# wangjiarui153/AIGV-Assessor

Measured on AMD Instinct MI355X. Metric: scored clips/sec (8-frame 448x448, InternVL2-8B stage-2 score eval), higher is better.
Workload: dtype bf16

## Files before the change

### aigv-assessor_amd/csrc/slowfast.hip

```cpp
#include <hip/hip_runtime.h>

#include <algorithm>
#include <cmath>
#include <cstdarg>
#include <cstdio>
#include <cstring>
#include <map>
#include <string>
#include <vector>

#include "../../include/aigv_amd.h"
#include "common.h"
#include "kernels.h"

namespace {

struct ConvArgs {
  const bf16_t* in;
  const bf16_t* w;
  const float* bias;
  const bf16_t* res;
  bf16_t* out;
  int ld_in, Cin, Ti, Hi, Wi;
  int kt, kh, kw, st, sh, sw, pt, ph, pw;
  int To, Ho, Wo, Cout, CoutPad, Kp;
  int ld_res, ld_out, c_off, relu;
  long rows;
  float* part;
  int k_slices;
};

template <int BN>
__global__ __launch_bounds__(256) void conv3d_mfma_kernel(ConvArgs p) {
  constexpr int BM = 128, BK = 64, NT = BN / 16, WJ = (BN + 31) / 32;
  __shared__ __attribute__((aligned(16))) bf16_t sA[BM * BK];
  __shared__ __attribute__((aligned(16))) bf16_t sW[BN * BK];
  const int tid = threadIdx.x, lane = tid & 63, wave = tid >> 6;
  const long m0 = (long)blockIdx.x * BM;
  const int n0 = blockIdx.y * BN;
  const int kspan = p.Kp / p.k_slices, kb = blockIdx.z * kspan;
  const int kc = tid & 7;
  const int r0 = tid >> 3;
  long base[4];
  int t0[4], y0[4], x0[4];
  bool rv[4];
#pragma unroll
  for (int j = 0; j < 4; ++j) {
    const long m = m0 + r0 + 32 * j;
    rv[j] = m < p.rows;
    const long mm = rv[j] ? m : 0;
    const int x = (int)(mm % p.Wo);
    const long r1 = mm / p.Wo;
    const int y = (int)(r1 % p.Ho);
    const long r2 = r1 / p.Ho;
    const int t = (int)(r2 % p.To);
    const long b = r2 / p.To;
    t0[j] = t * p.st - p.pt;
    y0[j] = y * p.sh - p.ph;
    x0[j] = x * p.sw - p.pw;
    base[j] = b * p.Ti * p.Hi * p.Wi;
  }
  int c = kb + kc * 8, dx = 0, dy = 0, dt = 0;
  auto normalise = [&]() {
    while (c >= p.Cin) {
      c -= p.Cin;
      if (++dx == p.kw) {
        dx = 0;
        if (++dy == p.kh) { dy = 0; ++dt; }
      }
    }
  };
  normalise();
  auto gather = [&](int j) -> u16x8 {
    u16x8 z = {0, 0, 0, 0, 0, 0, 0, 0};
    if (!rv[j] || dt >= p.kt) return z;
    const int tt = t0[j] + dt, yy = y0[j] + dy, xx = x0[j] + dx;
    if ((unsigned)tt >= (unsigned)p.Ti || (unsigned)yy >= (unsigned)p.Hi || (unsigned)xx >= (unsigned)p.Wi) return z;
    return *(const u16x8*)(p.in + (base[j] + ((long)tt * p.Hi + yy) * p.Wi + xx) * p.ld_in + c);
  };
  bool wv[WJ];
  const bf16_t* wsrc[WJ];
#pragma unroll
  for (int j = 0; j < WJ; ++j) {
    const int wrow = r0 + 32 * j;
    wv[j] = wrow < BN && (n0 + wrow) < p.CoutPad;
    wsrc[j] = p.w + (size_t)(n0 + (wv[j] ? wrow : 0)) * p.Kp + kb + kc * 8;
  }
  f32x4 acc[2][NT];
#pragma unroll
  for (int i = 0; i < 2; ++i)
#pragma unroll
    for (int n = 0; n < NT; ++n) acc[i][n] = f32x4{0.f, 0.f, 0.f, 0.f};

  const u16x8 zero = {0, 0, 0, 0, 0, 0, 0, 0};
  u16x8 ra[4], rw[WJ];
#pragma unroll
  for (int j = 0; j < 4; ++j) ra[j] = gather(j);
#pragma unroll
  for (int j = 0; j < WJ; ++j) rw[j] = wv[j] ? *(const u16x8*)wsrc[j] : zero;
  const int slot = (kc ^ (r0 & 7)) * 8;
  for (int k0 = 0; k0 < kspan; k0 += BK) {
    __syncthreads();
#pragma unroll
    for (int j = 0; j < 4; ++j) *(u16x8*)&sA[(r0 + 32 * j) * BK + slot] = ra[j];
#pragma unroll
    for (int j = 0; j < WJ; ++j)
      if (r0 + 32 * j < BN) *(u16x8*)&sW[(r0 + 32 * j) * BK + slot] = rw[j];
    __syncthreads();
    if (k0 + BK < kspan) {
      c += BK;
      normalise();
#pragma unroll
      for (int j = 0; j < 4; ++j) ra[j] = gather(j);
#pragma unroll
      for (int j = 0; j < WJ; ++j) rw[j] = wv[j] ? *(const u16x8*)(wsrc[j] + k0 + BK) : zero;
    }
#pragma unroll
    for (int h = 0; h < 2; ++h) {
      const int rs = ((h * 4 + (lane >> 4)) ^ (lane & 7)) * 8;
      bf16x8 a[2], w[NT];
#pragma unroll
      for (int i = 0; i < 2; ++i) a[i] = *(const bf16x8*)&sA[(wave * 32 + i * 16 + (lane & 15)) * BK + rs];
#pragma unroll
      for (int n = 0; n < NT; ++n) w[n] = *(const bf16x8*)&sW[(n * 16 + (lane & 15)) * BK + rs];
#pragma unroll
      for (int i = 0; i < 2; ++i)
#pragma unroll
        for (int n = 0; n < NT; ++n) acc[i][n] = __builtin_amdgcn_mfma_f32_16x16x32_bf16(w[n], a[i], acc[i][n], 0, 0, 0);
    }
  }
#pragma unroll
  for (int i = 0; i < 2; ++i) {
    const long m = m0 + wave * 32 + i * 16 + (lane & 15);
    if (m >= p.rows) continue;
#pragma unroll
    for (int n = 0; n < NT; ++n) {
      const int ch = n0 + n * 16 + (lane >> 4) * 4;
      if (ch >= p.Cout) continue;
      if (p.k_slices > 1) {
        *(f32x4*)(p.part + ((size_t)blockIdx.z * p.rows + m) * p.Cout + ch) = acc[i][n];
        continue;
      }
      float v[4];
#pragma unroll
      for (int e = 0; e < 4; ++e) v[e] = acc[i][n][e] + p.bias[ch + e];
      if (p.res) {
        const u16x4 r = *(const u16x4*)(p.res + m * p.ld_res + ch);
#pragma unroll
        for (int e = 0; e < 4; ++e) v[e] += bf2f(r[e]);
      }
      u16x4 o;
#pragma unroll
      for (int e = 0; e < 4; ++e) o[e] = f2bf(p.relu ? fmaxf(v[e], 0.f) : v[e]);
      *(u16x4*)(p.out + m * p.ld_out + p.c_off + ch) = o;
    }
  }
}

__global__ __launch_bounds__(256) void conv_finalize_kernel(ConvArgs p) {
  const long i = (long)blockIdx.x * 256 + threadIdx.x;
  const int cq = p.Cout >> 2;
  if (i >= p.rows * cq) return;
  const long m = i / cq;
  const int ch = (int)(i - m * cq) * 4;
  f32x4 v = *(const f32x4*)(p.part + (size_t)m * p.Cout + ch);
  for (int z = 1; z < p.k_slices; ++z) v += *(const f32x4*)(p.part + ((size_t)z * p.rows + m) * p.Cout + ch);
#pragma unroll
  for (int e = 0; e < 4; ++e) v[e] += p.bias[ch + e];
  if (p.res) {
    const u16x4 r = *(const u16x4*)(p.res + m * p.ld_res + ch);
#pragma unroll
    for (int e = 0; e < 4; ++e) v[e] += bf2f(r[e]);
  }
  u16x4 o;
#pragma unroll
  for (int e = 0; e < 4; ++e) o[e] = f2bf(p.relu ? fmaxf(v[e], 0.f) : v[e]);
  *(u16x4*)(p.out + m * p.ld_out + p.c_off + ch) = o;
}

struct FrameIdx { int v[64]; };
__global__ __launch_bounds__(256) void sf_repack_kernel(const bf16_t* __restrict__ frames, int T, int Ts, long hw, bf16_t* __restrict__ fast,
                                                        bf16_t* __restrict__ slow, FrameIdx idx, long total) {
  const long i = (long)blockIdx.x * 256 + threadIdx.x;
  if (i >= total) return;
  const long px = i % hw;
  const long f = i / hw;
  const int tt = (int)(f % (T + Ts));
  const long b = f / (T + Ts);
  const int src_t = tt < T ? tt : idx.v[tt - T];
  const bf16_t* s = frames + ((b * T + src_t) * 3) * hw + px;
  u16x4 o = {s[0], s[hw], s[2 * hw], 0};
  bf16_t* d = tt < T ? fast + ((b * T + tt) * hw + px) * 4 : slow + ((b * Ts + (tt - T)) * hw + px) * 4;
  *(u16x4*)d = o;
}

__global__ __launch_bounds__(256) void sf_maxpool_kernel(const bf16_t* __restrict__ in, int C, int Hi, int Wi, int Ho, int Wo,
                                                         bf16_t* __restrict__ out, int ld_out, long total) {
  const long i = (long)blockIdx.x * 256 + threadIdx.x;
  if (i >= total) return;
  const int cv = C >> 3;
  const int c8 = (int)(i % cv);
  const long px = i / cv;
  const int x = (int)(px % Wo);
  const long r = px / Wo;
  const int y = (int)(r % Ho);
  const long f = r / Ho;
  float m[8];
#pragma unroll
  for (int e = 0; e < 8; ++e) m[e] = -INFINITY;
  for (int dy = 0; dy < 3; ++dy) {
    const int yy = 2 * y - 1 + dy;
    if ((unsigned)yy >= (unsigned)Hi) continue;
    for (int dx = 0; dx < 3; ++dx) {
      const int xx = 2 * x - 1 + dx;
      if ((unsigned)xx >= (unsigned)Wi) continue;
      const u16x8 v = *(const u16x8*)(in + ((f * Hi + yy) * Wi + xx) * C + c8 * 8);
#pragma unroll
      for (int e = 0; e < 8; ++e) m[e] = fmaxf(m[e], bf2f(v[e]));
    }
  }
  u16x8 o;
#pragma unroll
  for (int e = 0; e < 8; ++e) o[e] = f2bf(m[e]);
  *(u16x8*)(out + px * ld_out + c8 * 8) = o;
}

struct PoolW { float t[32], y[32], x[32]; };
__global__ __launch_bounds__(256) void sf_pool_kernel(const bf16_t* __restrict__ in, int T, int H, int W, int C, PoolW w,
                                                      bf16_t* __restrict__ out, int ld_out, int c_off) {
  __shared__ float red[64][4][8];
  const int chunk = threadIdx.x & 3, slice = threadIdx.x >> 2;
  const int c8 = blockIdx.x * 4 + chunk;
  const int b = blockIdx.y;
  float acc[8] = {0.f, 0.f, 0.f, 0.f, 0.f, 0.f, 0.f, 0.f};
  if (c8 * 8 < C) {
    const bf16_t* s = in + (long)b * T * H * W * C + c8 * 8;
    const int n = T * H * W;
    for (int i = slice; i < n; i += 64) {
      const int x = i % W, r = i / W, y = r % H, t = r / H;
      const float wt = w.t[t] * w.y[y] * w.x[x];
      const u16x8 v = *(const u16x8*)(s + (long)i * C);
#pragma unroll
      for (int e = 0; e < 8; ++e) acc[e] += wt * bf2f(v[e]);
    }
  }
#pragma unroll
  for (int e = 0; e < 8; ++e) red[slice][chunk][e] = acc[e];
  __syncthreads();
  if (threadIdx.x < 32 && (blockIdx.x * 4 + (threadIdx.x >> 3)) * 8 < C) {
    const int ch = threadIdx.x >> 3, e = threadIdx.x & 7;
    float v = 0.f;
    for (int q = 0; q < 64; ++q) v += red[q][ch][e];
    out[(long)b * ld_out + c_off + (blockIdx.x * 4 + ch) * 8 + e] = f2bf(v);
  }
}

constexpr long SPLITK_MAX_ROWS = 8192;

int conv_k_slices(long rows, int CoutPad, int Kp) {
  if (rows > SPLITK_MAX_ROWS || Kp < 1024) return 1;
  const int bn = CoutPad >= 64 ? 64 : CoutPad >= 32 ? 32 : 16;
  const long tiles = ((rows + 127) / 128) * ((CoutPad + bn - 1) / bn);
  if (tiles >= 64) return 1;
  const int steps = Kp / 64;
  for (int S : {8, 6, 4, 3, 2})
    if (steps % S == 0 && steps / S >= 4 && tiles * S <= 512) return S;
  return 1;
}

hipError_t launch_conv(const ConvArgs& a_in, hipStream_t s, int S = 1, float* ws = nullptr, size_t ws_floats = 0) {
  ConvArgs a = a_in;
  if (a.rows <= 0) return hipSuccess;
  if (a.Cin % 8 || a.ld_in % 8 || a.Cout % 4 || a.ld_out % 4 || a.c_off % 4 || a.Kp % 64 || a.CoutPad % 16 || (a.res && a.ld_res % 4) ||
      a.Kp < a.kt * a.kh * a.kw * a.Cin)
    return hipErrorInvalidValue;
  if (!ws || S < 1 || (a.Kp / 64) % S || (size_t)S * a.rows * a.Cout > ws_floats) S = 1;
  a.k_slices = S;
  a.part = S > 1 ? ws : nullptr;
  const unsigned gx = (unsigned)((a.rows + 127) / 128);
  if (a.CoutPad >= 64) hipLaunchKernelGGL(conv3d_mfma_kernel<64>, dim3(gx, (a.CoutPad + 63) / 64, S), dim3(256), 0, s, a);
  else if (a.CoutPad >= 32) hipLaunchKernelGGL(conv3d_mfma_kernel<32>, dim3(gx, (a.CoutPad + 31) / 32, S), dim3(256), 0, s, a);
  else hipLaunchKernelGGL(conv3d_mfma_kernel<16>, dim3(gx, 1, S), dim3(256), 0, s, a);
  if (S > 1) {
    const long total = a.rows * (a.Cout / 4);
    hipLaunchKernelGGL(conv_finalize_kernel, dim3((unsigned)((total + 255) / 256)), dim3(256), 0, s, a);
  }
  return hipGetLastError();
}

inline uint16_t bf16_host(float f) {
  uint32_t u;
  memcpy(&u, &f, 4);
  if ((u & 0x7fffffffu) > 0x7f800000u) return (uint16_t)((u >> 16) | 0x40);
  u += 0x7fffu + ((u >> 16) & 1u);
  return (uint16_t)(u >> 16);
}
inline float bf16_to_float_host(uint16_t h) {
  uint32_t u = (uint32_t)h << 16;
  float f;
  memcpy(&f, &u, 4);
  return f;
}

struct HostTensor {
  std::vector<float> v;
  std::vector<int64_t> shape;
};

enum OpKind { OP_REPACK, OP_CONV, OP_MAXPOOL, OP_POOL };
struct Op {
  OpKind kind;
  ConvArgs a{};
  int in_buf = -1, out_buf = -1, res_buf = -1;
  size_t w_off = 0, b_off = 0;
  long rows_per_clip = 0;
  int k_slices = 1;
  int C = 0, T = 0, Hi = 0, Wi = 0, Ho = 0, Wo = 0, ld_out = 0, c_off = 0;
  PoolW pw{};
};

int sf_fail(int code, const char* fmt, ...) {
  char buf[768];
  va_list ap;
  va_start(ap, fmt);
  vsnprintf(buf, sizeof buf, fmt, ap);
  va_end(ap);
  aigv_set_error(buf);
  return code;
}

}

struct aigv_slowfast {
  int device = 0, Bcap = 0, T = 0, Ts = 0, H = 0, W = 0;
  bool finalized = false;
  std::map<std::string, HostTensor> host;
  std::vector<Op> ops;
  std::vector<size_t> buf_elems;
  std::vector<bf16_t*> bufs;
  bf16_t* d_w = nullptr;
  float* d_b = nullptr;
  float* d_part = nullptr;
  size_t part_floats = 0;
  FrameIdx slow_idx{};
  double flops_per_clip = 0;
};

namespace {

enum { B_IN0 = 0, B_IN1, B_STEM0, B_STEM1, B_X00, B_X01, B_X10, B_X11, B_A0, B_A1, B_B0, B_B1, B_S0, B_S1, B_COUNT };

struct Builder {
  aigv_slowfast* sf;
  std::vector<uint16_t> w;
  std::vector<float> b;
  std::string missing;

  const HostTensor* get(const std::string& name) {
    auto it = sf->host.find(name);
    if (it == sf->host.end()) {
      if (missing.size() < 400) missing += (missing.empty() ? "" : ", ") + name;
      return nullptr;
    }
    return &it->second;
  }
  void need(int buf, size_t elems) {
    if (sf->buf_elems[buf] < elems) sf->buf_elems[buf] = elems;
  }
  bool conv(const std::string& conv_name, const std::string& norm_name, int in_buf, int ld_in, int cin_eff, int Ti, int Hi, int Wi, int kt, int kh,
            int kw, int st, int sh, int sw, int pt, int ph, int pw, int cout, int out_buf, int ld_out, int c_off, int res_buf, int ld_res, bool relu,
            int* To_, int* Ho_, int* Wo_, bool stem_pairs = false) {
    const HostTensor* W = get(conv_name + ".weight");
    const HostTensor* g = get(norm_name + ".weight");
    const HostTensor* be = get(norm_name + ".bias");
    const HostTensor* mu = get(norm_name + ".running_mean");
    const HostTensor* var = get(norm_name + ".running_var");
    const int To = (Ti + 2 * pt - kt) / st + 1, Ho = (Hi + 2 * ph - kh) / sh + 1, Wo = (Wi + 2 * pw - kw) / sw + 1;
    *To_ = To; *Ho_ = Ho; *Wo_ = Wo;
    if (!W || !g || !be || !mu || !var) return false;
    const int cin_real = W->shape.size() == 5 ? (int)W->shape[1] : -1;
    if (W->shape.size() != 5 || W->shape[0] != cout || (stem_pairs ? cin_real != 3 : cin_real != cin_eff) || W->shape[2] != kt || W->shape[3] != kh || W->shape[4] != kw ||
        (int)g->v.size() != cout || (int)be->v.size() != cout || (int)mu->v.size() != cout || (int)var->v.size() != cout) {
      if (missing.size() < 400) missing += (missing.empty() ? "" : ", ") + conv_name + " (bad shape)";
      return false;
    }
    const int taps = kt * kh * kw;
    const int kw_k = stem_pairs ? 4 : kw, taps_k = kt * kh * kw_k;
    const int K = taps_k * cin_eff, Kp = (K + 63) / 64 * 64, coutPad = (cout + 15) / 16 * 16;
    Op op;
    op.kind = OP_CONV;
    op.w_off = w.size();
    op.b_off = b.size();
    w.resize(w.size() + (size_t)coutPad * Kp, 0);
    b.resize(b.size() + cout, 0.f);
    for (int co = 0; co < cout; ++co) {
      const float scale = g->v[co] / std::sqrt(var->v[co] + 1e-5f);
      b[op.b_off + co] = be->v[co] - mu->v[co] * scale;
      uint16_t* dst = &w[op.w_off + (size_t)co * Kp];
      for (int ci = 0; ci < cin_real; ++ci)
        for (int tap = 0; tap < taps; ++tap) {
          int k = tap * cin_eff + ci;
          if (stem_pairs) {
            const int q = tap % kw + 1;
            k = ((tap / kw) * 4 + (q >> 1)) * 8 + (q & 1) * 4 + ci;
          }
          dst[k] = bf16_host(W->v[((size_t)co * cin_real + ci) * taps + tap] * scale);
        }
    }
    ConvArgs& a = op.a;
    a.ld_in = ld_in; a.Cin = cin_eff; a.Ti = Ti; a.Hi = Hi; a.Wi = stem_pairs ? Wi / 2 : Wi;
    a.kt = kt; a.kh = kh; a.kw = kw_k; a.st = st; a.sh = sh; a.sw = stem_pairs ? 1 : sw; a.pt = pt; a.ph = ph; a.pw = stem_pairs ? 2 : pw;
    a.To = To; a.Ho = Ho; a.Wo = Wo; a.Cout = cout; a.CoutPad = coutPad; a.Kp = Kp;
    a.ld_res = ld_res; a.ld_out = ld_out; a.c_off = c_off; a.relu = relu ? 1 : 0;
    op.in_buf = in_buf; op.out_buf = out_buf; op.res_buf = res_buf;
    op.rows_per_clip = (long)To * Ho * Wo;
    need(out_buf, (size_t)op.rows_per_clip * ld_out);
    sf->flops_per_clip += 2.0 * op.rows_per_clip * cout * (double)taps * cin_real;
    sf->ops.push_back(op);
    return true;
  }
};

void cover_weights(float* w, int n, int k) {
  for (int i = 0; i < n; ++i) {
    const int lo = i - k + 1 > 0 ? i - k + 1 : 0, hi = i < n - k ? i : n - k;
    w[i] = (float)(hi - lo + 1);
  }
}

}

extern "C" {

int aigv_slowfast_create(int device, int max_clips, int frames_per_clip, int height, int width, aigv_slowfast** out) {
  if (!out) return sf_fail(AIGV_ERR_ARG, "aigv_slowfast_create: null argument");
  *out = nullptr;
  int ndev = 0;
  if (hipGetDeviceCount(&ndev) != hipSuccess || ndev <= 0)
    return sf_fail(AIGV_ERR_HIP, "aigv_slowfast_create: no HIP device is visible (this library has no CPU fallback)");
  if (device < 0 || device >= ndev) return sf_fail(AIGV_ERR_ARG, "aigv_slowfast_create: device %d out of range (%d visible)", device, ndev);
  if (max_clips <= 0 || frames_per_clip < 8 || frames_per_clip > 32 || frames_per_clip % 4 || height < 224 || width < 224 || height % 32 ||
      width % 32 || height > 1024 || width > 1024)
    return sf_fail(AIGV_ERR_ARG, "aigv_slowfast_create: needs 8 <= T <= 32 with T %% 4 == 0 and 224 <= H, W <= 1024 multiples of 32 (got T=%d %dx%d)",
                   frames_per_clip, height, width);
  aigv_slowfast* sf = new (std::nothrow) aigv_slowfast();
  if (!sf) return sf_fail(AIGV_ERR_ALLOC, "out of host memory");
  sf->device = device; sf->Bcap = max_clips; sf->T = frames_per_clip; sf->Ts = frames_per_clip / 4; sf->H = height; sf->W = width;
  const int n = sf->Ts;
  const float step = n > 1 ? (float)(sf->T - 1) / (float)(n - 1) : 0.f;
  for (int i = 0; i < n; ++i) sf->slow_idx.v[i] = i < n / 2 ? (int)(0.f + step * i) : (int)((float)(sf->T - 1) - step * (float)(n - 1 - i));
  *out = sf;
  return 0;
}

void aigv_slowfast_destroy(aigv_slowfast* sf) {
  if (!sf) return;
  hipSetDevice(sf->device);
  hipDeviceSynchronize();
  for (bf16_t* p : sf->bufs) hipFree(p);
  hipFree(sf->d_w);
  hipFree(sf->d_b);
  hipFree(sf->d_part);
  delete sf;
}

int aigv_slowfast_load_weight(aigv_slowfast* sf, const char* name, const void* host_data, const int64_t* shape, int ndim, int dtype) {
  if (!sf || !name || !host_data || !shape || ndim <= 0 || ndim > 5) return sf_fail(AIGV_ERR_ARG, "aigv_slowfast_load_weight: bad argument");
  if (sf->finalized) return sf_fail(AIGV_ERR_STATE, "aigv_slowfast_load_weight(%s): already finalized", name);
  std::string key(name);
  for (const char* pre : {"slowfast_model.feature_extraction.", "feature_extraction.", "blocks."}) {
    const size_t n = strlen(pre);
    if (key.compare(0, n, pre) == 0) { key = key.substr(n); break; }
  }
  HostTensor t;
  size_t n = 1;
  for (int i = 0; i < ndim; ++i) {
    if (shape[i] <= 0) return sf_fail(AIGV_ERR_ARG, "aigv_slowfast_load_weight(%s): bad shape", name);
    n *= (size_t)shape[i];
    t.shape.push_back(shape[i]);
  }
  t.v.resize(n);
  if (dtype == AIGV_F32) memcpy(t.v.data(), host_data, n * 4);
  else if (dtype == AIGV_BF16) for (size_t i = 0; i < n; ++i) t.v[i] = bf16_to_float_host(((const uint16_t*)host_data)[i]);
  else return sf_fail(AIGV_ERR_ARG, "aigv_slowfast_load_weight(%s): dtype %d", name, dtype);
  sf->host[key] = std::move(t);
  return 0;
}

int aigv_slowfast_finalize(aigv_slowfast* sf) {
  if (!sf) return sf_fail(AIGV_ERR_ARG, "aigv_slowfast_finalize: null handle");
  if (sf->finalized) return 0;
  if (hipSetDevice(sf->device) != hipSuccess) return sf_fail(AIGV_ERR_HIP, "hipSetDevice failed");
  sf->ops.clear();
  sf->buf_elems.assign(B_COUNT, 0);
  sf->flops_per_clip = 0;
  Builder bd{sf, {}, {}, {}};
  const int T[2] = {sf->Ts, sf->T};
  const int IN[2] = {B_IN0, B_IN1}, STEM[2] = {B_STEM0, B_STEM1}, X[2][2] = {{B_X00, B_X01}, {B_X10, B_X11}}, A[2] = {B_A0, B_A1},
            Bq[2] = {B_B0, B_B1}, S[2] = {B_S0, B_S1};
  {
    Op op; op.kind = OP_REPACK;
    sf->ops.push_back(op);
    bd.need(B_IN0, (size_t)sf->Ts * sf->H * sf->W * 4);
    bd.need(B_IN1, (size_t)sf->T * sf->H * sf->W * 4);
  }
  bool ok = true;
  int h = 0, w = 0, to = 0;
  int ld[2] = {64 + 16, 8};
  for (int p = 0; p < 2; ++p) {
    const int kt = p ? 5 : 1, cout = p ? 8 : 64;
    const std::string pre = "0.multipathway_blocks." + std::to_string(p);
    ok &= bd.conv(pre + ".conv", pre + ".norm", IN[p], 8, 8, T[p], sf->H, sf->W, kt, 7, 7, 1, 2, 2, kt / 2, 3, 3, cout, STEM[p], cout, 0, -1, 0, true, &to, &h, &w, true);
    Op mp; mp.kind = OP_MAXPOOL;
    mp.in_buf = STEM[p]; mp.out_buf = X[p][0]; mp.C = cout; mp.T = T[p]; mp.Hi = h; mp.Wi = w;
    mp.Ho = (h + 2 - 3) / 2 + 1; mp.Wo = (w + 2 - 3) / 2 + 1; mp.ld_out = ld[p];
    bd.need(X[p][0], (size_t)T[p] * mp.Ho * mp.Wo * ld[p]);
    sf->ops.push_back(mp);
    if (p == 1) { h = mp.Ho; w = mp.Wo; }
  }
  int sp_h = h, sp_w = w;
  ok &= bd.conv("0.multipathway_fusion.conv_fast_to_slow", "0.multipathway_fusion.norm", X[1][0], 8, 8, T[1], sp_h, sp_w, 7, 1, 1, 4, 1, 1, 3, 0, 0, 16,
                X[0][0], ld[0], 64, -1, 0, true, &to, &h, &w);
  if (to != T[0]) return sf_fail(AIGV_ERR_ARG, "fast->slow fusion yields %d frames, slow pathway has %d", to, T[0]);
  int cur[2] = {0, 0};
  int cin[2] = {80, 8};
  static const int depths[4] = {3, 4, 6, 3};
  for (int s = 0; s < 4; ++s) {
    int out_h = sp_h, out_w = sp_w;
    for (int p = 0; p < 2; ++p) {
      const int inner = (p ? 8 : 64) << s, cout = inner * 4;
      const int fuse_ch = (s < 3 && p == 0) ? 2 * (32 << s) : 0;
      const int ld_out = cout + fuse_ch;
      const int kt_a = (p == 1 || s >= 2) ? 3 : 1;
      int bh = sp_h, bw = sp_w;
      for (int blk = 0; blk < depths[s]; ++blk) {
        const int stv = (blk == 0 && s > 0) ? 2 : 1;
        const std::string pre = std::to_string(s + 1) + ".multipathway_blocks." + std::to_string(p) + ".res_blocks." + std::to_string(blk) + ".";
        const int xin = X[p][cur[p]], xout = X[p][cur[p] ^ 1];
        const int c_in = blk == 0 ? cin[p] : cout, ld_in = blk == 0 ? ld[p] : ld_out;
        int t1, h1, w1, h2, w2;
        int res_buf = xin, res_ld = ld_in;
        if (blk == 0) {
          ok &= bd.conv(pre + "branch1_conv", pre + "branch1_norm", xin, ld_in, c_in, T[p], bh, bw, 1, 1, 1, 1, stv, stv, 0, 0, 0, cout, S[p], cout, 0, -1, 0,
                        false, &t1, &h1, &w1);
          res_buf = S[p]; res_ld = cout;
        }
        ok &= bd.conv(pre + "branch2.conv_a", pre + "branch2.norm_a", xin, ld_in, c_in, T[p], bh, bw, kt_a, 1, 1, 1, 1, 1, kt_a / 2, 0, 0, inner, A[p], inner, 0,
                      -1, 0, true, &t1, &h1, &w1);
        ok &= bd.conv(pre + "branch2.conv_b", pre + "branch2.norm_b", A[p], inner, inner, T[p], bh, bw, 1, 3, 3, 1, stv, stv, 0, 1, 1, inner, Bq[p], inner, 0, -1,
                      0, true, &t1, &h2, &w2);
        ok &= bd.conv(pre + "branch2.conv_c", pre + "branch2.norm_c", Bq[p], inner, inner, T[p], h2, w2, 1, 1, 1, 1, 1, 1, 0, 0, 0, cout, xout, ld_out, 0, res_buf,
                      res_ld, true, &t1, &h1, &w1);
        bh = h2; bw = w2;
        cur[p] ^= 1;
      }
      cin[p] = ld_out; ld[p] = ld_out;
      out_h = bh; out_w = bw;
    }
    sp_h = out_h; sp_w = out_w;
    if (s < 3) {
      const int cf = 32 << s, cs = 256 << s;
      const std::string pre = std::to_string(s + 1) + ".multipathway_fusion";
      ok &= bd.conv(pre + ".conv_fast_to_slow", pre + ".norm", X[1][cur[1]], cf, cf, T[1], sp_h, sp_w, 7, 1, 1, 4, 1, 1, 3, 0, 0, 2 * cf, X[0][cur[0]], ld[0], cs,
                    -1, 0, true, &to, &h, &w);
    }
  }
  if (!ok) return sf_fail(AIGV_ERR_STATE, "aigv_slowfast_finalize: missing or mis-shaped tensors: %s%s", bd.missing.c_str(), bd.missing.size() >= 400 ? " ..." : "");
  if (sp_h < 7 || sp_w < 7 || sp_h > 32 || sp_w > 32) return sf_fail(AIGV_ERR_ARG, "final map %dx%d outside the head pool's range", sp_h, sp_w);
  for (int p = 0; p < 2; ++p) {
    Op op; op.kind = OP_POOL;
    op.in_buf = X[p][cur[p]]; op.C = p ? 256 : 2048; op.T = T[p]; op.Hi = sp_h; op.Wi = sp_w; op.ld_out = 2304; op.c_off = p ? 2048 : 0;
    const int L = 4 * T[p], k = p ? 32 : 8;
    if (L < k) return sf_fail(AIGV_ERR_ARG, "too few frames for the head pool");
    float rep[128];
    cover_weights(rep, L, k);
    float ty[32], tx[32];
    cover_weights(ty, sp_h, 7);
    cover_weights(tx, sp_w, 7);
    const float nt = (float)(L - k + 1) * k, ny = (float)(sp_h - 6) * 7, nx = (float)(sp_w - 6) * 7;
    for (int t = 0; t < T[p]; ++t) op.pw.t[t] = (rep[4 * t] + rep[4 * t + 1] + rep[4 * t + 2] + rep[4 * t + 3]) / nt;
    for (int y = 0; y < sp_h; ++y) op.pw.y[y] = ty[y] / ny;
    for (int x = 0; x < sp_w; ++x) op.pw.x[x] = tx[x] / nx;
    sf->ops.push_back(op);
  }
  auto dmalloc = [&](void** p, size_t bytes) { return hipMalloc(p, bytes ? bytes : 16); };
  if (dmalloc((void**)&sf->d_w, bd.w.size() * 2) != hipSuccess || dmalloc((void**)&sf->d_b, bd.b.size() * 4) != hipSuccess)
    return sf_fail(AIGV_ERR_ALLOC, "aigv_slowfast_finalize: hipMalloc of %zu weight bytes failed", bd.w.size() * 2);
  if (hipMemcpy(sf->d_w, bd.w.data(), bd.w.size() * 2, hipMemcpyHostToDevice) != hipSuccess ||
      hipMemcpy(sf->d_b, bd.b.data(), bd.b.size() * 4, hipMemcpyHostToDevice) != hipSuccess)
    return sf_fail(AIGV_ERR_HIP, "aigv_slowfast_finalize: weight upload failed");
  sf->bufs.assign(B_COUNT, nullptr);
  for (int i = 0; i < B_COUNT; ++i) {
    const size_t bytes = sf->buf_elems[i] * (size_t)sf->Bcap * 2 + 64;
    if (hipMalloc((void**)&sf->bufs[i], bytes) != hipSuccess) return sf_fail(AIGV_ERR_ALLOC, "aigv_slowfast_finalize: hipMalloc(%zu) failed", bytes);
    if (hipMemset(sf->bufs[i], 0, bytes) != hipSuccess) return sf_fail(AIGV_ERR_HIP, "hipMemset failed");
  }
  size_t need = 0;
  for (Op& op : sf->ops) {
    if (op.kind != OP_CONV) continue;
    op.k_slices = conv_k_slices(op.rows_per_clip, op.a.CoutPad, op.a.Kp);
    if (op.k_slices > 1) need = std::max(need, (size_t)op.k_slices * op.rows_per_clip * sf->Bcap * op.a.Cout);
  }
  sf->part_floats = need;
  if (sf->part_floats && hipMalloc((void**)&sf->d_part, sf->part_floats * sizeof(float)) != hipSuccess)
    return sf_fail(AIGV_ERR_ALLOC, "aigv_slowfast_finalize: hipMalloc of the split-K workspace failed");
  sf->host.clear();
  sf->finalized = true;
  return 0;
}

double aigv_slowfast_flops_per_clip(const aigv_slowfast* sf) { return sf ? sf->flops_per_clip : 0.0; }

int aigv_slowfast_forward(aigv_slowfast* sf, const void* frames_nchw_bf16, int clips, void* feature_bf16, void* stream) {
  if (!sf || !frames_nchw_bf16 || !feature_bf16) return sf_fail(AIGV_ERR_ARG, "aigv_slowfast_forward: null argument");
  if (!sf->finalized) return sf_fail(AIGV_ERR_STATE, "aigv_slowfast_forward: call aigv_slowfast_finalize first");
  if (clips <= 0 || clips > sf->Bcap) return sf_fail(AIGV_ERR_ARG, "aigv_slowfast_forward: %d clips, capacity %d", clips, sf->Bcap);
  if (hipSetDevice(sf->device) != hipSuccess) return sf_fail(AIGV_ERR_HIP, "aigv_slowfast_forward: hipSetDevice(%d) failed", sf->device);
  hipStream_t s = (hipStream_t)stream;
  for (const Op& op : sf->ops) {
    hipError_t e = hipSuccess;
    switch (op.kind) {
      case OP_REPACK: {
        const long hw = (long)sf->H * sf->W, total = (long)clips * (sf->T + sf->Ts) * hw;
        hipLaunchKernelGGL(sf_repack_kernel, dim3((unsigned)((total + 255) / 256)), dim3(256), 0, s, (const bf16_t*)frames_nchw_bf16, sf->T, sf->Ts, hw,
                           sf->bufs[B_IN1], sf->bufs[B_IN0], sf->slow_idx, total);
        e = hipGetLastError();
        break;
      }
      case OP_CONV: {
        ConvArgs a = op.a;
        a.in = sf->bufs[op.in_buf]; a.out = sf->bufs[op.out_buf]; a.res = op.res_buf >= 0 ? sf->bufs[op.res_buf] : nullptr;
        a.w = sf->d_w + op.w_off; a.bias = sf->d_b + op.b_off;
        a.rows = op.rows_per_clip * clips;
        e = launch_conv(a, s, op.k_slices, sf->d_part, sf->part_floats);
        break;
      }
      case OP_MAXPOOL: {
        const long total = (long)clips * op.T * op.Ho * op.Wo * (op.C / 8);
        hipLaunchKernelGGL(sf_maxpool_kernel, dim3((unsigned)((total + 255) / 256)), dim3(256), 0, s, sf->bufs[op.in_buf], op.C, op.Hi, op.Wi, op.Ho, op.Wo,
                           sf->bufs[op.out_buf], op.ld_out, total);
        e = hipGetLastError();
        break;
      }
      case OP_POOL: {
        hipLaunchKernelGGL(sf_pool_kernel, dim3((op.C + 31) / 32, clips), dim3(256), 0, s, sf->bufs[op.in_buf], op.T, op.Hi, op.Wi, op.C, op.pw,
                           (bf16_t*)feature_bf16, op.ld_out, op.c_off);
        e = hipGetLastError();
        break;
      }
    }
    if (e != hipSuccess) return sf_fail(e == hipErrorInvalidValue ? AIGV_ERR_ARG : AIGV_ERR_HIP, "aigv_slowfast_forward: launch failed: %s", hipGetErrorString(e));
  }
  return 0;
}

int aigv_op_conv3d(const void* x, int ld_in, int Cin, int B, const int* dims, const void* w_packed, int Kp, const float* bias, int Cout, const void* res,
                   int ld_res, void* out, int ld_out, int c_off, int relu, void* stream) {
  if (!x || !dims || !w_packed || !bias || !out) return sf_fail(AIGV_ERR_ARG, "aigv_op_conv3d: null argument");
  ConvArgs a{};
  a.in = (const bf16_t*)x; a.ld_in = ld_in; a.Cin = Cin; a.Ti = dims[0]; a.Hi = dims[1]; a.Wi = dims[2];
  a.kt = dims[3]; a.kh = dims[4]; a.kw = dims[5]; a.st = dims[6]; a.sh = dims[7]; a.sw = dims[8]; a.pt = dims[9]; a.ph = dims[10]; a.pw = dims[11];
  if (a.kt <= 0 || a.kh <= 0 || a.kw <= 0 || a.st <= 0 || a.sh <= 0 || a.sw <= 0 || a.pt < 0 || a.ph < 0 || a.pw < 0 || B <= 0 || Cin <= 0 || Cout <= 0 ||
      ld_in < Cin || ld_out < c_off + Cout || (res && ld_res < Cout) || a.Ti + 2 * a.pt < a.kt || a.Hi + 2 * a.ph < a.kh || a.Wi + 2 * a.pw < a.kw)
    return sf_fail(AIGV_ERR_ARG, "aigv_op_conv3d: bad geometry");
  a.To = (a.Ti + 2 * a.pt - a.kt) / a.st + 1; a.Ho = (a.Hi + 2 * a.ph - a.kh) / a.sh + 1; a.Wo = (a.Wi + 2 * a.pw - a.kw) / a.sw + 1;
  a.w = (const bf16_t*)w_packed; a.Kp = Kp; a.bias = bias; a.Cout = Cout; a.CoutPad = (Cout + 15) / 16 * 16;
  a.res = (const bf16_t*)res; a.ld_res = ld_res; a.out = (bf16_t*)out; a.ld_out = ld_out; a.c_off = c_off; a.relu = relu;
  a.rows = (long)B * a.To * a.Ho * a.Wo;
  hipError_t e = launch_conv(a, (hipStream_t)stream);
  if (e != hipSuccess)
    return sf_fail(e == hipErrorInvalidValue ? AIGV_ERR_ARG : AIGV_ERR_HIP,
                   "aigv_op_conv3d (Cin=%d Cout=%d Kp=%d; needs Cin, ld_in %% 8 == 0, Cout, ld_out, c_off %% 4 == 0, Kp %% 64 == 0): %s", Cin, Cout, Kp, hipGetErrorString(e));
  return 0;
}

}
```

### aigv-assessor_amd/native.py

```python
from __future__ import annotations

import ctypes as C
import os
from typing import Optional

HERE = os.path.dirname(os.path.abspath(__file__))
LIB_PATH = os.environ.get("AIGV_AMD_LIB") or os.path.join(HERE, "libaigv_amd.so")
ABI_VERSION = 3


class NativeError(RuntimeError):
    pass


class AigvConfig(C.Structure):
    _fields_ = [
        ("vit_hidden", C.c_int32), ("vit_inter", C.c_int32), ("vit_heads", C.c_int32), ("vit_layers", C.c_int32),
        ("image_size", C.c_int32), ("patch_size", C.c_int32), ("num_channels", C.c_int32),
        ("vit_norm_rms", C.c_int32), ("vit_qk_norm", C.c_int32), ("vit_qkv_bias", C.c_int32),
        ("vit_eps", C.c_float), ("select_layer", C.c_int32), ("shuffle", C.c_int32),
        ("llm_hidden", C.c_int32), ("llm_inter", C.c_int32), ("llm_heads", C.c_int32), ("llm_kv_heads", C.c_int32),
        ("llm_layers", C.c_int32), ("vocab", C.c_int32), ("rms_eps", C.c_float), ("max_positions", C.c_int32),
        ("motion_dim", C.c_int32), ("n_score_layers", C.c_int32), ("score_dims", C.c_int32 * 8),
        ("max_frames", C.c_int32), ("vit_chunk", C.c_int32), ("max_tokens", C.c_int32), ("max_seqs", C.c_int32),
        ("max_out_rows", C.c_int32), ("kv_capacity", C.c_int32),
    ]


_P = C.c_void_p
_I = C.c_int
_F = C.c_float
_I64P = C.POINTER(C.c_int64)
_I32P = C.POINTER(C.c_int32)

PROTOTYPES = {
    "aigv_abi_version": (_I, []),
    "aigv_sizeof_config": (_I, []),
    "aigv_ctx_create": (_I, [_I, C.POINTER(AigvConfig), C.POINTER(_P)]),
    "aigv_ctx_destroy": (None, [_P]),
    "aigv_ctx_resize": (_I, [_P, C.POINTER(AigvConfig)]),
    "aigv_last_error": (C.c_char_p, [_P]),
    "aigv_clear_hip_error": (None, []),
    "aigv_load_weight": (_I, [_P, C.c_char_p, _P, _I64P, _I, _I, _I]),
    "aigv_finalize_weights": (_I, [_P]),
    "aigv_vit_forward": (_I, [_P, _P, _I, _P, _P]),
    "aigv_project": (_I, [_P, _P, _I, _P, _P]),
    "aigv_motion_project": (_I, [_P, _P, _I, _P, _P]),
    "aigv_llm_prefill": (_I, [_P, _P, _P, _I32P, _I, _P, _I, _P, _I32P, _P, _I32P, _I, _P, _I, _P]),
    "aigv_llm_extend": (_I, [_P, _P, _I32P, _I, _I32P, _P, _I32P, _I, _P, _I, _P]),
    "aigv_kv_fork": (_I, [_P, _I, _P]),
    "aigv_kv_reorder": (_I, [_P, _P, _P, _I, _P]),
    "aigv_set_row_trimming": (_I, [_P, _I]),
    "aigv_set_gemm_mode": (_I, [_P, _I]),
    "aigv_set_attention_numerics": (_I, [_P, _I]),
    "aigv_get_attention_numerics": (_I, [_P]),
    "aigv_ctx_tune": (_I, [_P, _I, _I]),
    "aigv_decode_step": (_I, [_P, _P, _P, _P]),
    "aigv_decode_step_logprob": (_I, [_P, _P, _P, _P, _P]),
    "aigv_out_row_logits": (_I, [_P, _I, _I, _P, _I, _P]),
    "aigv_out_row_hidden": (_I, [_P, _I, _I, _P, _I, _P]),
    "aigv_out_row_logprob": (_I, [_P, _I, _I, _P, _P, _P]),
    "aigv_decode_eos": (_I, [_P, _P, _P, _I64P, _I, C.c_int64, _P]),
    "aigv_op_gemm": (_I, [_P, _I, _P, _I, _P, _I, _P, _P, _P, _I, _P, _I, _I, _I, _I, _I, _P]),
    "aigv_op_gemm_rows": (_I, [_P, _I, _P, _I, _P, _I, _P, _P, _P, _I, C.POINTER(C.c_int32), _I, _I, _I, _I, _P]),
    "aigv_op_gemm_splitk": (_I, [_P, _I, _P, _I, _P, _I, _P, _P, _P, _I, _I, _I, _I, _I, _I, _P, _P]),
    "aigv_op_gemm_splitk256": (_I, [_P, _I, _P, _I, _P, _I, _P, _P, _P, _I, _I, _I, _I, _I, _I, _P, _P]),
    "aigv_slowfast_create": (_I, [_I, _I, _I, _I, _I, C.POINTER(_P)]),
    "aigv_slowfast_destroy": (None, [_P]),
    "aigv_slowfast_load_weight": (_I, [_P, C.c_char_p, _P, C.POINTER(C.c_int64), _I, _I]),
    "aigv_slowfast_finalize": (_I, [_P]),
    "aigv_slowfast_forward": (_I, [_P, _P, _I, _P, _P]),
    "aigv_slowfast_flops_per_clip": (C.c_double, [_P]),
    "aigv_op_conv3d": (_I, [_P, _I, _I, _I, C.POINTER(_I), _P, _I, _P, _I, _P, _I, _P, _I, _I, _I, _P]),
    "aigv_set_precision": (_I, [_P, _I]),
    "aigv_op_quant_fp8_rows": (_I, [_P, _I, _I, _I, _P, _I, _P, _P]),
    "aigv_op_gemm_fp8": (_I, [_P, _I, _P, _I, _P, _I, _P, _P, _P, _P, _P, _I, _I, _I, _I, _I, _I, _P, _P]),
    "aigv_op_skinny_gemm": (_I, [_P, _I, _I, _P, _I, _I, _I, _P, _P, _I, _P, _I, _I, _P]),
    "aigv_op_skinny_gemm_fp8": (_I, [_P, _I, _I, _P, _I, C.POINTER(C.c_float), _I, _I, _P, _I, _P, _I, _I, _P, _F, _I, _P]),
    "aigv_op_layernorm": (_I, [_P, _I, _P, _P, _P, _I, _I, _I, _F, _P]),
    "aigv_op_rmsnorm": (_I, [_P, _I, _P, _P, _I, _I, _I, _F, _P, _P]),
    "aigv_op_rope": (_I, [_P, _I, _P, _P, _P, _I, _I, _I, _I, _I, _P]),
    "aigv_op_attention": (_I, [_P, _I, _P, _I, _P, _I, _P, _I, _P, _I, _I, _I, _I, _I, _I, _I, _I, _F, _F, _P]),
    "aigv_op_attention_rope": (_I, [_P, _I, _P, _I, _P, _I, _P, _I, _P, _I, _I, _I, _I, _I, _I, _I, _I, _F, _F, _P, _P, _P, _P]),
    "aigv_op_pixel_shuffle": (_I, [_P, _I, _I, _P, _I, _P]),
    "aigv_op_im2col": (_I, [_P, _I, _I, _I, _I, _I, _P, _P]),
    "aigv_op_lm_head_argmax": (_I, [_P, _I, _I, _P, _I, _P, _P, _P, _P]),
    "aigv_op_lm_head_argmax_logprob": (_I, [_P, _I, _I, _P, _I, _P, C.c_int64, _P, _P, _P, _P]),
    "aigv_op_lm_head_argmax_logprob_scratch_bytes": (C.c_int64, [_I, _I]),
    "aigv_op_label_logprob": (_I, [_P, _I, _I, _I, _P, _P, _P]),
    "aigv_op_attention_decode": (_I, [_P, _I, _I, _P, _P, _P, _I, _P, _I, _I, _I, _I, _I, _F, _I, _P, C.c_int64, _P]),
    "aigv_op_attention_decode_ws_floats": (C.c_int64, [_I, _I, _I, _I]),
    "aigv_op_skinny_rope_kv": (_I, [_P, _I, _I, _P, _I, _I, _I, _P, _I, _P, _P, _P, _P, _P, _P, _I, _I, _I, _P, _F, _I, _P]),
    "aigv_op_skinny_swiglu_normed": (_I, [_P, _I, _I, _P, _I, _I, _I, _P, _I, _P, _F, _I, _P]),
    "aigv_op_skinny_rope_kv_fp8": (_I, [_P, _I, _I, _P, _I, _P, _I, _I, _P, _I, _P, _P, _P, _P, _P, _P, _I, _I, _I, _P, _F, _I, _P]),
    "aigv_op_frame_ingest": (_I, [_P, _I, _I, _I, C.POINTER(C.c_float), C.POINTER(C.c_float), _P, _P]),
    "aigv_op_frame_resize_ingest": (_I, [_P, _I, _I, _I, _I, _I, C.POINTER(C.c_float), C.POINTER(C.c_float), _P, _P, _P, _P]),
    "aigv_tune_gemm": (_I, [_I, C.c_double]),
    "aigv_tune_co_gemm": (_I, [_I]),
    "aigv_tune_default": (_I, [_I, _I]),
    "aigv_tune_attention": (_I, [_I]),
    "aigv_tune_skinny": (_I, [_I]),
    "aigv_plan_gemm": (_I, [_I, _I, _I, _I, C.POINTER(C.c_int), C.POINTER(C.c_double)]),
    "aigv_prof_enable": (_I, [_P, _I]),
    "aigv_prof_read": (_I, [_P, _I, _I64P, C.POINTER(C.c_double), C.POINTER(C.c_double), C.POINTER(C.c_double)]),
}

_lib: Optional[C.CDLL] = None


def load() -> C.CDLL:
    global _lib
    if _lib is not None:
        return _lib
    if not os.path.exists(LIB_PATH):
        raise NativeError(f"{LIB_PATH} not found: the HIP extension is not built (run __graft_entry__.build()); "
                          "there is no CPU fallback for the product path")
    import torch
    lib = C.CDLL(LIB_PATH)
    for name, (res, args) in PROTOTYPES.items():
        try:
            fn = getattr(lib, name)
        except AttributeError:
            raise NativeError(f"ABI mismatch: {LIB_PATH} does not match binding ABI {ABI_VERSION} (rebuild it): missing {name}") from None
        fn.restype = res
        fn.argtypes = args
    if lib.aigv_abi_version() != ABI_VERSION:
        raise NativeError(f"ABI mismatch: library {lib.aigv_abi_version()} vs binding {ABI_VERSION}")
    if lib.aigv_sizeof_config() != C.sizeof(AigvConfig):
        raise NativeError(f"aigv_config layout mismatch: C {lib.aigv_sizeof_config()} vs ctypes {C.sizeof(AigvConfig)}")
    _lib = lib
    return lib


def check(rc: int, ctx=None):
    if rc != 0:
        msg = load().aigv_last_error(ctx)
        raise NativeError(f"libaigv_amd error {rc}: {msg.decode() if msg else '?'}")


def ptr(t) -> Optional[int]:
    if t is None:
        return None
    assert t.is_contiguous(), "native ops take contiguous tensors"
    return t.data_ptr()


def stream_ptr() -> Optional[int]:
    import torch
    s = torch.cuda.current_stream().cuda_stream
    return s if s else None


def i32_array(values):
    arr = (C.c_int32 * len(values))(*[int(v) for v in values])
    return arr


import contextlib
import gc

_captures_underway = 0
_deferred_releases = []


def release(fn_name: str, handle) -> None:
    if handle is None:
        return
    capturing = _captures_underway > 0
    if not capturing:
        try:
            import torch
            capturing = torch.cuda.is_available() and torch.cuda.is_current_stream_capturing()
        except Exception:
            capturing = False
    if capturing:
        _deferred_releases.append((fn_name, handle))
    else:
        getattr(load(), fn_name)(handle)


def flush_releases() -> None:
    while _deferred_releases and _captures_underway == 0:
        fn_name, handle = _deferred_releases.pop()
        getattr(load(), fn_name)(handle)


@contextlib.contextmanager
def capturing():
    global _captures_underway
    gc.collect()
    was_enabled = gc.isenabled()
    gc.disable()
    _captures_underway += 1
    try:
        yield
    finally:
        _captures_underway -= 1
        if was_enabled:
            gc.enable()
        flush_releases()
```

### aigv-assessor_amd/slowfast.py

```python
from __future__ import annotations

import collections
import ctypes as C
import itertools
from typing import Dict, Iterator, Optional, Tuple

import torch

from . import native

PREFIX = "slowfast_model.feature_extraction."
FEATURE_DIM = 2304


_UIDS = itertools.count(1)


class SlowFastR50:
    MAX_HANDLES = 8

    def __init__(self, state_dict: Optional[Dict[str, torch.Tensor]] = None):
        self._sd: Dict[str, torch.Tensor] = {}
        self._handles: "collections.OrderedDict[Tuple, Tuple[int, int]]" = collections.OrderedDict()
        self._handle: Optional[int] = None
        self.epoch = 0
        self.uid = next(_UIDS)
        if state_dict is not None:
            self.load_state_dict(state_dict)

    def load_state_dict(self, state_dict: Dict[str, torch.Tensor], strict: bool = True):
        sd = {}
        for k, v in state_dict.items():
            for pre in (PREFIX, "feature_extraction.", "blocks."):
                if k.startswith(pre):
                    k = k[len(pre):]
                    break
            if k.endswith("num_batches_tracked") or not k[:1].isdigit():
                continue
            if int(k.split(".", 1)[0]) > 4:
                continue
            sd[k] = v.detach().to(device="cpu", dtype=torch.float32).contiguous()
        if strict and not sd:
            raise RuntimeError("no SlowFast tensors in the state dict")
        self._sd = sd
        self._release()

    def state_dict(self, prefix: str = PREFIX) -> Dict[str, torch.Tensor]:
        return {prefix + k: v for k, v in self._sd.items()}

    def parameters(self) -> Iterator[torch.nn.Parameter]:
        for v in self._sd.values():
            yield torch.nn.Parameter(v, requires_grad=False)

    def eval(self):
        return self

    def _destroy(self, handle):
        self.epoch += 1
        native.release("aigv_slowfast_destroy", handle)

    def _release(self):
        for h, _cap in list(self._handles.values()):
            self._destroy(h)
        self._handles.clear()
        self._handle = None

    def __del__(self):
        try:
            self._release()
        except Exception:
            pass

    def prepare(self, device: torch.device, clips: int, T: int, H: int, W: int):
        lib = native.load()
        dev = device.index if device.index is not None else torch.cuda.current_device()
        key = (dev, T, H, W)
        ent = self._handles.get(key)
        if ent is not None and ent[1] >= clips:
            self._handles.move_to_end(key)
            self._handle = ent[0]
            return lib, ent[0]
        if native._captures_underway > 0 or torch.cuda.is_current_stream_capturing():
            raise RuntimeError(f"SlowFastR50: no native handle for {clips} clips of {T} x {H} x {W} yet and one cannot be created inside a stream capture "
                               "(call prepare() before capturing)")
        if not self._sd:
            raise RuntimeError("SlowFastR50 has no weights: load_state_dict() first")
        if ent is not None:
            del self._handles[key]
            self._destroy(ent[0])
        while len(self._handles) >= self.MAX_HANDLES:
            _k, (h_old, _cap) = self._handles.popitem(last=False)
            self._destroy(h_old)
        h = C.c_void_p()
        native.check(lib.aigv_slowfast_create(dev, clips, T, H, W, C.byref(h)))
        try:
            for name, t in self._sd.items():
                shape = (C.c_int64 * t.dim())(*t.shape)
                native.check(lib.aigv_slowfast_load_weight(h, name.encode(), t.data_ptr(), shape, t.dim(), 1))
            native.check(lib.aigv_slowfast_finalize(h))
        except Exception:
            lib.aigv_slowfast_destroy(h)
            raise
        self._handles[key] = (h, clips)
        self._handle = h
        return lib, h

    def _native(self, device: torch.device, clips: int, T: int, H: int, W: int):
        return self.prepare(device, clips, T, H, W)

    def features(self, pixel_values: torch.Tensor, clips: int) -> torch.Tensor:
        if not pixel_values.is_cuda:
            raise RuntimeError("SlowFastR50 runs on the GPU only (no CPU fallback)")
        if pixel_values.dim() != 4 or pixel_values.shape[1] != 3 or clips <= 0 or pixel_values.shape[0] % clips:
            raise ValueError(f"pixel_values must be [clips * T, 3, H, W]; got {tuple(pixel_values.shape)} for {clips} clips")
        T, H, W = pixel_values.shape[0] // clips, pixel_values.shape[2], pixel_values.shape[3]
        x = pixel_values.to(torch.bfloat16).contiguous()
        lib, h = self._native(x.device, clips, T, H, W)
        out = torch.empty((clips, FEATURE_DIM), dtype=torch.bfloat16, device=x.device)
        native.check(lib.aigv_slowfast_forward(h, x.data_ptr(), clips, out.data_ptr(), native.stream_ptr()))
        return out

    def flops_per_clip(self) -> float:
        return float(native.load().aigv_slowfast_flops_per_clip(self._handle)) if self._handle is not None else 0.0

    def __call__(self, inputs) -> torch.Tensor:
        fast = inputs[1]
        B, _, T, H, W = fast.shape
        frames = fast.permute(0, 2, 1, 3, 4).reshape(B * T, 3, H, W)
        return self.features(frames, B).view(B, FEATURE_DIM, 1, 1, 1)
```

### include/aigv_amd.h

```cpp
#ifndef AIGV_AMD_H
#define AIGV_AMD_H

#include <stdint.h>

#ifdef __cplusplus
extern "C" {
#endif

#define AIGV_ABI_VERSION 3

#define AIGV_MAX_KV_CAPACITY 262144

typedef struct aigv_ctx aigv_ctx;

enum aigv_status {
  AIGV_OK = 0,
  AIGV_ERR_ARG = -1,
  AIGV_ERR_HIP = -2,
  AIGV_ERR_STATE = -3,
  AIGV_ERR_ALLOC = -4
};

enum aigv_dtype { AIGV_BF16 = 0, AIGV_F32 = 1 };

typedef struct aigv_config {
  int32_t vit_hidden, vit_inter, vit_heads, vit_layers;
  int32_t image_size, patch_size, num_channels;
  int32_t vit_norm_rms;
  int32_t vit_qk_norm;
  int32_t vit_qkv_bias;
  float vit_eps;
  int32_t select_layer;
  int32_t shuffle;
  int32_t llm_hidden, llm_inter, llm_heads, llm_kv_heads, llm_layers, vocab;
  float rms_eps;
  int32_t max_positions;
  int32_t motion_dim;
  int32_t n_score_layers;
  int32_t score_dims[8];
  int32_t max_frames;
  int32_t vit_chunk;
  int32_t max_tokens;
  int32_t max_seqs;
  int32_t max_out_rows;
  int32_t kv_capacity;
} aigv_config;

int aigv_abi_version(void);
int aigv_sizeof_config(void);
int aigv_ctx_create(int device, const aigv_config* cfg, aigv_ctx** out);
void aigv_ctx_destroy(aigv_ctx* ctx);
int aigv_ctx_resize(aigv_ctx* ctx, const aigv_config* cfg);
const char* aigv_last_error(const aigv_ctx* ctx);
void aigv_clear_hip_error(void);

int aigv_load_weight(aigv_ctx* ctx, const char* name, const void* data, const int64_t* shape, int ndim,
                     int dtype, int on_device);
int aigv_finalize_weights(aigv_ctx* ctx);

int aigv_vit_forward(aigv_ctx* ctx, const void* frames, int n_frames, void* out_tokens, void* stream);
int aigv_project(aigv_ctx* ctx, const void* tokens, int rows, void* out, void* stream);
int aigv_motion_project(aigv_ctx* ctx, const void* motion_feature, int n_clips, void* out, void* stream);

int aigv_llm_prefill(aigv_ctx* ctx, const int64_t* ids, const int32_t* slot, const int32_t* cu_seqlens, int n_clips,
                     const void* vis, int n_vis, const void* motion, const int32_t* score_rows, float* score,
                     const int32_t* logit_rows, int n_logit_rows, int64_t* argmax, int keep_kv, void* stream);
int aigv_llm_extend(aigv_ctx* ctx, const int64_t* ids, const int32_t* cu, int n_clips, const int32_t* score_rows, float* score,
                    const int32_t* logit_rows, int n_logit_rows, int64_t* argmax, int commit, void* stream);

int aigv_kv_fork(aigv_ctx* ctx, int copies, void* stream);
int aigv_kv_reorder(aigv_ctx* ctx, const int32_t* parent, const int32_t* len, int n, void* stream);

enum aigv_precision { AIGV_PRECISION_BF16 = 0, AIGV_PRECISION_FP8_LLM = 1 };
int aigv_set_precision(aigv_ctx* ctx, int mode);
int aigv_set_row_trimming(aigv_ctx* ctx, int on);
#define AIGV_ATTENTION_NUMERICS_DEFAULT 0
int aigv_set_attention_numerics(aigv_ctx* ctx, int mode);
int aigv_get_attention_numerics(const aigv_ctx* ctx);
int aigv_set_gemm_mode(aigv_ctx* ctx, int mode);

int aigv_decode_step(aigv_ctx* ctx, const int64_t* ids, int64_t* next, void* stream);
int aigv_decode_step_logprob(aigv_ctx* ctx, const int64_t* ids, int64_t* next, float* logprob, void* stream);
int aigv_out_row_logits(aigv_ctx* ctx, int first_row, int n_rows, void* logits_bf16, int ldo, void* stream);
int aigv_out_row_hidden(aigv_ctx* ctx, int first_row, int n_rows, void* hidden_bf16, int ldo, void* stream);
int aigv_out_row_logprob(aigv_ctx* ctx, int first_row, int n_rows, const int64_t* labels, float* logprob, void* stream);
int aigv_decode_eos(aigv_ctx* ctx, int64_t* tokens, int32_t* state, const int64_t* eos_ids, int n_eos, int64_t pad_id, void* stream);

int aigv_op_gemm(const void* A, int lda, const void* W, int ldw, void* C, int ldc, const void* bias, const void* ls,
                 const void* resid, int ldr, const void* pos, int np, int M, int N, int K, int epi, void* stream);
int aigv_op_gemm_rows(const void* A, int lda, const void* W, int ldw, void* C, int ldc, const void* bias, const void* ls,
                      const void* resid, int ldr, const int32_t* cu_host, int n_seq, int N, int K, int epi, void* stream);
int aigv_op_gemm_splitk(const void* A, int lda, const void* W, int ldw, void* C, int ldc, const void* bias, const void* ls,
                        const void* resid, int ldr, int M, int N, int K, int epi, int k_slices, void* ws_f32, void* stream);
int aigv_op_gemm_splitk256(const void* A, int lda, const void* W, int ldw, void* C, int ldc, const void* bias, const void* ls,
                           const void* resid, int ldr, int M, int N, int K, int epi, int k_slices, void* ws_f32, void* stream);
int aigv_op_quant_fp8_rows(const void* x_bf16, int ldx, int rows, int K, void* q_e4m3, int ldq, float* row_scale, void* stream);
int aigv_op_gemm_fp8(const void* A_e4m3, int lda, const void* W_e4m3, int ldw, void* C, int ldc, const float* row_scale,
                     const float* col_scale, const void* bias, const void* ls, const void* resid, int ldr, int M, int N, int K, int epi,
                     int k_slices, void* ws_f32, void* stream);
int aigv_op_skinny_gemm(const void* x, int ldx, int R, const void* W, int ldw, int N, int K, const void* bias,
                        const void* resid, int ldr, void* out, int ldo, int epi, void* stream);
int aigv_op_skinny_gemm_fp8(const void* x, int ldx, int R, const void* W_e4m3, int ldw, const float* w_scale, int N, int K, const void* resid,
                            int ldr, void* out, int ldo, int epi, const void* norm_w, float eps, int p, void* stream);
int aigv_op_layernorm(const void* x, int ldx, const void* w, const void* b, void* y, int ldy, int rows, int H,
                      float eps, void* stream);
int aigv_op_rmsnorm(const void* x, int ldx, const void* w, void* y, int ldy, int rows, int H, float eps,
                    const int32_t* row_idx, void* stream);
int aigv_op_rope(void* qkv, int ld, const int32_t* pos, const void* cos, const void* sin, int tokens, int n_rot,
                 int slots, int n_groups, int head_dim, void* stream);
int aigv_op_attention(const void* q, int ldq, const void* k, int ldk, const void* v, int ldv, void* o, int ldo,
                      const int32_t* cu, int n_seq, int max_len, int n_heads, int n_kv_heads, int q_group_stride,
                      int kv_head_stride, int head_dim, int causal, float post_div, float q_prescale, void* stream);
int aigv_op_attention_rope(const void* q, int ldq, const void* k, int ldk, const void* v, int ldv, void* o, int ldo,
                           const int32_t* cu, int n_seq, int max_len, int n_heads, int n_kv_heads, int q_group_stride,
                           int kv_head_stride, int head_dim, int causal, float post_div, float q_prescale, const int32_t* pos,
                           const void* cos, const void* sin, void* stream);
int aigv_op_pixel_shuffle(const void* vit_out, int grid, int vit_hidden, void* out, int n_frames, void* stream);
int aigv_op_im2col(const void* frames, int n_frames, int channels, int image_size, int patch, int kp, void* out,
                   void* stream);
int aigv_op_lm_head_argmax(const void* h, int rows, int hidden, const void* W, int vocab, void* scratch_u64,
                           int64_t* idx, float* val, void* stream);
int aigv_op_lm_head_argmax_logprob(const void* h, int rows, int hidden, const void* W, int vocab, void* scratch, int64_t scratch_bytes,
                                   int64_t* idx, float* val, float* logprob, void* stream);
int64_t aigv_op_lm_head_argmax_logprob_scratch_bytes(int rows, int vocab);
int aigv_op_label_logprob(const void* logits_bf16, int rows, int vocab, int ldo, const int64_t* labels, float* out, void* stream);

int aigv_op_attention_decode(const void* q, int ldq, int q_group_stride, const void* kc, const void* vc, const int32_t* kv_lens, int cap,
                             void* o, int ldo, int n_seq, int n_kv, int g, int head_dim, float post_div, int max_kv_len, float* ws,
                             int64_t ws_floats, void* stream);
int64_t aigv_op_attention_decode_ws_floats(int n_seq, int n_kv, int g, int cap);
int aigv_op_skinny_rope_kv(const void* x, int ldx, int R, const void* W, int ldw, int N, int K, void* qkv, int ldo, const int32_t* pos,
                           const int32_t* seq, const void* cos, const void* sin, void* kc, void* vc, int g, int n_kv, int cap,
                           const void* norm_w, float eps, int p, void* stream);
int aigv_op_skinny_swiglu_normed(const void* x, int ldx, int R, const void* W, int ldw, int N, int K, void* out, int ldo,
                                 const void* norm_w, float eps, int p, void* stream);
int aigv_op_skinny_rope_kv_fp8(const void* x, int ldx, int R, const void* W_e4m3, int ldw, const float* w_scale, int N, int K, void* qkv,
                               int ldo, const int32_t* pos, const int32_t* seq, const void* cos, const void* sin, void* kc, void* vc, int g,
                               int n_kv, int cap, const void* norm_w, float eps, int p, void* stream);

int aigv_op_frame_ingest(const void* hwc_u8, int n_frames, int height, int width, const float* mean, const float* stdv,
                         void* out_nchw, void* stream);

int aigv_op_frame_resize_ingest(const void* hwc_u8, int n_frames, int in_h, int in_w, int out_h, int out_w, const float* mean,
                                const float* stdv, void* tmp_u8, void* out_u8_hwc, void* out_nchw, void* stream);

enum aigv_tune_knob {
  AIGV_TUNE_GEMM_MODE = 0,
  AIGV_TUNE_GEMM256_ORDER = 1,
  AIGV_TUNE_GEMM256_VARIANT = 2,
  AIGV_TUNE_ATTN_WAVES = 3,
  AIGV_TUNE_SKINNY_P = 4,
  AIGV_TUNE_BODY_TILE = 5,
  AIGV_TUNE_CO_KMAX = 6,
  AIGV_TUNE_TAIL_SLICES = 7,
  AIGV_TUNE_ATTN_LEAD_KEY = 8,
  AIGV_TUNE_DECODE_FUSED = 9,
  AIGV_TUNE_DECODE_FP8 = 10,
  AIGV_TUNE_SKINNY_P8 = 11,
  AIGV_TUNE_FUSE_TAILS = 12,
  AIGV_TUNE_LONE_BODY = 13,
  AIGV_TUNE_COUNT = 14
};
int aigv_ctx_tune(aigv_ctx* ctx, int knob, int value);
int aigv_tune_gemm(int mode, double rate256);
int aigv_tune_co_gemm(int kmax);
int aigv_tune_default(int knob, int value);
int aigv_plan_gemm(int M, int N, int K, int epi, int* plan, double* est_us);
int aigv_tune_attention(int waves);
int aigv_tune_skinny(int p);

enum aigv_prof_class { AIGV_PROF_GEMM = 0, AIGV_PROF_ATTN_VIT = 1, AIGV_PROF_ATTN_LLM = 2, AIGV_PROF_SKINNY = 3,
                       AIGV_PROF_GEMM_FP8 = 4, AIGV_PROF_GEMM_VIT = 5, AIGV_PROF_COUNT = 6 };
int aigv_prof_enable(aigv_ctx* ctx, int on);
int aigv_prof_read(aigv_ctx* ctx, int cls, int64_t* launches, double* total_ms, double* flops, double* bytes);

typedef struct aigv_slowfast aigv_slowfast;
int aigv_slowfast_create(int device, int max_clips, int frames_per_clip, int height, int width, aigv_slowfast** out);
void aigv_slowfast_destroy(aigv_slowfast* sf);
int aigv_slowfast_load_weight(aigv_slowfast* sf, const char* name, const void* host_data, const int64_t* shape, int ndim, int dtype);
int aigv_slowfast_finalize(aigv_slowfast* sf);
int aigv_slowfast_forward(aigv_slowfast* sf, const void* frames_nchw_bf16, int clips, void* feature_bf16, void* stream);
double aigv_slowfast_flops_per_clip(const aigv_slowfast* sf);
int aigv_op_conv3d(const void* x, int ld_in, int Cin, int B, const int* dims, const void* w_packed, int Kp, const float* bias, int Cout,
                   const void* res, int ld_res, void* out, int ld_out, int c_off, int relu, void* stream);

#ifdef __cplusplus
}
#endif
#endif
```

Measured before the change: 33.57.

## Fuse slow and fast SlowFast pathway kernels into paired launches

```diff
diff --git a/aigv-assessor_amd/csrc/slowfast.hip b/aigv-assessor_amd/csrc/slowfast.hip
--- a/aigv-assessor_amd/csrc/slowfast.hip
+++ b/aigv-assessor_amd/csrc/slowfast.hip
@@ -31,14 +31,12 @@
 };
 
 template <int BN>
-__global__ __launch_bounds__(256) void conv3d_mfma_kernel(ConvArgs p) {
+__device__ __forceinline__ void conv_tile(const ConvArgs& p, int bx, int by, int bz, bf16_t* __restrict__ sA, bf16_t* __restrict__ sW) {
   constexpr int BM = 128, BK = 64, NT = BN / 16, WJ = (BN + 31) / 32;
-  __shared__ __attribute__((aligned(16))) bf16_t sA[BM * BK];
-  __shared__ __attribute__((aligned(16))) bf16_t sW[BN * BK];
   const int tid = threadIdx.x, lane = tid & 63, wave = tid >> 6;
-  const long m0 = (long)blockIdx.x * BM;
-  const int n0 = blockIdx.y * BN;
-  const int kspan = p.Kp / p.k_slices, kb = blockIdx.z * kspan;
+  const long m0 = (long)bx * BM;
+  const int n0 = by * BN;
+  const int kspan = p.Kp / p.k_slices, kb = bz * kspan;
   const int kc = tid & 7;
   const int r0 = tid >> 3;
   long base[4];
@@ -138,7 +136,7 @@
       const int ch = n0 + n * 16 + (lane >> 4) * 4;
       if (ch >= p.Cout) continue;
       if (p.k_slices > 1) {
-        *(f32x4*)(p.part + ((size_t)blockIdx.z * p.rows + m) * p.Cout + ch) = acc[i][n];
+        *(f32x4*)(p.part + ((size_t)bz * p.rows + m) * p.Cout + ch) = acc[i][n];
         continue;
       }
       float v[4];
@@ -154,6 +152,31 @@
       for (int e = 0; e < 4; ++e) o[e] = f2bf(p.relu ? fmaxf(v[e], 0.f) : v[e]);
       *(u16x4*)(p.out + m * p.ld_out + p.c_off + ch) = o;
     }
+  }
+}
+
+template <int BN>
+__global__ __launch_bounds__(256) void conv3d_mfma_kernel(ConvArgs p) {
+  __shared__ __attribute__((aligned(16))) bf16_t sA[128 * 64];
+  __shared__ __attribute__((aligned(16))) bf16_t sW[BN * 64];
+  conv_tile<BN>(p, blockIdx.x, blockIdx.y, blockIdx.z, sA, sW);
+}
+
+struct ConvPair {
+  ConvArgs a[2];
+  unsigned gx[2], gy[2], nb[2];
+};
+template <int BN0, int BN1>
+__global__ __launch_bounds__(256) void conv3d_pair_kernel(ConvPair q) {
+  constexpr int BNM = BN0 > BN1 ? BN0 : BN1;
+  __shared__ __attribute__((aligned(16))) bf16_t sA[128 * 64];
+  __shared__ __attribute__((aligned(16))) bf16_t sW[BNM * 64];
+  const unsigned b = blockIdx.x;
+  if (b < q.nb[0]) {
+    conv_tile<BN0>(q.a[0], b % q.gx[0], (b / q.gx[0]) % q.gy[0], b / (q.gx[0] * q.gy[0]), sA, sW);
+  } else {
+    const unsigned l = b - q.nb[0];
+    conv_tile<BN1>(q.a[1], l % q.gx[1], (l / q.gx[1]) % q.gy[1], l / (q.gx[1] * q.gy[1]), sA, sW);
   }
 }
 
@@ -194,10 +217,23 @@
   *(u16x4*)d = o;
 }
 
-__global__ __launch_bounds__(256) void sf_maxpool_kernel(const bf16_t* __restrict__ in, int C, int Hi, int Wi, int Ho, int Wo,
-                                                         bf16_t* __restrict__ out, int ld_out, long total) {
-  const long i = (long)blockIdx.x * 256 + threadIdx.x;
-  if (i >= total) return;
+struct MaxPoolArgs {
+  const bf16_t* in;
+  bf16_t* out;
+  int C, Hi, Wi, Ho, Wo, ld_out;
+  long total;
+};
+struct MaxPoolPair {
+  MaxPoolArgs m[2];
+  unsigned nb0;
+};
+__global__ __launch_bounds__(256) void sf_maxpool_kernel(MaxPoolPair q) {
+  const bool second = blockIdx.x >= q.nb0;
+  const MaxPoolArgs& a = second ? q.m[1] : q.m[0];
+  const bf16_t* __restrict__ in = a.in;
+  const int C = a.C, Hi = a.Hi, Wi = a.Wi, Ho = a.Ho, Wo = a.Wo;
+  const long i = (long)(blockIdx.x - (second ? q.nb0 : 0)) * 256 + threadIdx.x;
+  if (i >= a.total) return;
   const int cv = C >> 3;
   const int c8 = (int)(i % cv);
   const long px = i / cv;
@@ -222,15 +258,29 @@
   u16x8 o;
 #pragma unroll
   for (int e = 0; e < 8; ++e) o[e] = f2bf(m[e]);
-  *(u16x8*)(out + px * ld_out + c8 * 8) = o;
+  *(u16x8*)(a.out + px * a.ld_out + c8 * 8) = o;
 }
 
 struct PoolW { float t[32], y[32], x[32]; };
-__global__ __launch_bounds__(256) void sf_pool_kernel(const bf16_t* __restrict__ in, int T, int H, int W, int C, PoolW w,
-                                                      bf16_t* __restrict__ out, int ld_out, int c_off) {
+struct PoolArgs {
+  const bf16_t* in;
+  int T, H, W, C, ld_out, c_off;
+  PoolW w;
+};
+struct PoolPair {
+  PoolArgs p[2];
+  unsigned nb0;
+};
+__global__ __launch_bounds__(256) void sf_pool_kernel(PoolPair q, bf16_t* __restrict__ out) {
   __shared__ float red[64][4][8];
+  const bool second = blockIdx.x >= q.nb0;
+  const PoolArgs& a = second ? q.p[1] : q.p[0];
+  const bf16_t* __restrict__ in = a.in;
+  const int T = a.T, H = a.H, W = a.W, C = a.C, ld_out = a.ld_out, c_off = a.c_off;
+  const PoolW& w = a.w;
+  const int bx = blockIdx.x - (second ? q.nb0 : 0);
   const int chunk = threadIdx.x & 3, slice = threadIdx.x >> 2;
-  const int c8 = blockIdx.x * 4 + chunk;
+  const int c8 = bx * 4 + chunk;
   const int b = blockIdx.y;
   float acc[8] = {0.f, 0.f, 0.f, 0.f, 0.f, 0.f, 0.f, 0.f};
   if (c8 * 8 < C) {
@@ -247,11 +297,11 @@
 #pragma unroll
   for (int e = 0; e < 8; ++e) red[slice][chunk][e] = acc[e];
   __syncthreads();
-  if (threadIdx.x < 32 && (blockIdx.x * 4 + (threadIdx.x >> 3)) * 8 < C) {
+  if (threadIdx.x < 32 && (bx * 4 + (threadIdx.x >> 3)) * 8 < C) {
     const int ch = threadIdx.x >> 3, e = threadIdx.x & 7;
     float v = 0.f;
-    for (int q = 0; q < 64; ++q) v += red[q][ch][e];
-    out[(long)b * ld_out + c_off + (blockIdx.x * 4 + ch) * 8 + e] = f2bf(v);
+    for (int s = 0; s < 64; ++s) v += red[s][ch][e];
+    out[(long)b * ld_out + c_off + (bx * 4 + ch) * 8 + e] = f2bf(v);
   }
 }
 
@@ -268,23 +318,73 @@
   return 1;
 }
 
+int conv_bn(int CoutPad) { return CoutPad >= 64 ? 64 : CoutPad >= 32 ? 32 : 16; }
+
+bool conv_args_ok(const ConvArgs& a) {
+  return !(a.Cin % 8 || a.ld_in % 8 || a.Cout % 4 || a.ld_out % 4 || a.c_off % 4 || a.Kp % 64 || a.CoutPad % 16 || (a.res && a.ld_res % 4) ||
+           a.Kp < a.kt * a.kh * a.kw * a.Cin);
+}
+
+size_t conv_split(ConvArgs& a, int S, float* ws, size_t ws_floats) {
+  if (!ws || S < 1 || (a.Kp / 64) % S || (size_t)S * a.rows * a.Cout > ws_floats) S = 1;
+  a.k_slices = S;
+  a.part = S > 1 ? ws : nullptr;
+  return S > 1 ? (size_t)S * a.rows * a.Cout : 0;
+}
+
+void launch_finalize(const ConvArgs& a, hipStream_t s) {
+  if (a.k_slices <= 1) return;
+  const long total = a.rows * (a.Cout / 4);
+  hipLaunchKernelGGL(conv_finalize_kernel, dim3((unsigned)((total + 255) / 256)), dim3(256), 0, s, a);
+}
+
 hipError_t launch_conv(const ConvArgs& a_in, hipStream_t s, int S = 1, float* ws = nullptr, size_t ws_floats = 0) {
   ConvArgs a = a_in;
   if (a.rows <= 0) return hipSuccess;
-  if (a.Cin % 8 || a.ld_in % 8 || a.Cout % 4 || a.ld_out % 4 || a.c_off % 4 || a.Kp % 64 || a.CoutPad % 16 || (a.res && a.ld_res % 4) ||
-      a.Kp < a.kt * a.kh * a.kw * a.Cin)
-    return hipErrorInvalidValue;
-  if (!ws || S < 1 || (a.Kp / 64) % S || (size_t)S * a.rows * a.Cout > ws_floats) S = 1;
-  a.k_slices = S;
-  a.part = S > 1 ? ws : nullptr;
+  if (!conv_args_ok(a)) return hipErrorInvalidValue;
+  conv_split(a, S, ws, ws_floats);
+  S = a.k_slices;
   const unsigned gx = (unsigned)((a.rows + 127) / 128);
   if (a.CoutPad >= 64) hipLaunchKernelGGL(conv3d_mfma_kernel<64>, dim3(gx, (a.CoutPad + 63) / 64, S), dim3(256), 0, s, a);
   else if (a.CoutPad >= 32) hipLaunchKernelGGL(conv3d_mfma_kernel<32>, dim3(gx, (a.CoutPad + 31) / 32, S), dim3(256), 0, s, a);
   else hipLaunchKernelGGL(conv3d_mfma_kernel<16>, dim3(gx, 1, S), dim3(256), 0, s, a);
-  if (S > 1) {
-    const long total = a.rows * (a.Cout / 4);
-    hipLaunchKernelGGL(conv_finalize_kernel, dim3((unsigned)((total + 255) / 256)), dim3(256), 0, s, a);
-  }
+  launch_finalize(a, s);
+  return hipGetLastError();
+}
+
+template <int BN0>
+void launch_pair_bn(const ConvPair& q, int bn1, hipStream_t s) {
+  const dim3 grid(q.nb[0] + q.nb[1]);
+  if (bn1 == 64) hipLaunchKernelGGL((conv3d_pair_kernel<BN0, 64>), grid, dim3(256), 0, s, q);
+  else if (bn1 == 32) hipLaunchKernelGGL((conv3d_pair_kernel<BN0, 32>), grid, dim3(256), 0, s, q);
+  else hipLaunchKernelGGL((conv3d_pair_kernel<BN0, 16>), grid, dim3(256), 0, s, q);
+}
+
+hipError_t launch_conv_pair(const ConvArgs& a0, int S0, const ConvArgs& a1, int S1, hipStream_t s, float* ws, size_t ws_floats) {
+  if (a0.rows <= 0 || a1.rows <= 0) {
+    const hipError_t e = launch_conv(a0, s, S0, ws, ws_floats);
+    return e != hipSuccess ? e : launch_conv(a1, s, S1, ws, ws_floats);
+  }
+  if (!conv_args_ok(a0) || !conv_args_ok(a1)) return hipErrorInvalidValue;
+  ConvPair q;
+  q.a[0] = a0;
+  q.a[1] = a1;
+  const size_t used = conv_split(q.a[0], S0, ws, ws_floats);
+  conv_split(q.a[1], S1, ws ? ws + used : nullptr, ws_floats - used);
+  auto work = [](const ConvArgs& a) { return (double)a.rows * a.CoutPad * a.Kp; };
+  if (work(q.a[1]) > work(q.a[0])) std::swap(q.a[0], q.a[1]);
+  int bn[2];
+  for (int i = 0; i < 2; ++i) {
+    bn[i] = conv_bn(q.a[i].CoutPad);
+    q.gx[i] = (unsigned)((q.a[i].rows + 127) / 128);
+    q.gy[i] = (unsigned)((q.a[i].CoutPad + bn[i] - 1) / bn[i]);
+    q.nb[i] = q.gx[i] * q.gy[i] * q.a[i].k_slices;
+  }
+  if (bn[0] == 64) launch_pair_bn<64>(q, bn[1], s);
+  else if (bn[0] == 32) launch_pair_bn<32>(q, bn[1], s);
+  else launch_pair_bn<16>(q, bn[1], s);
+  launch_finalize(q.a[0], s);
+  launch_finalize(q.a[1], s);
   return hipGetLastError();
 }
 
@@ -318,6 +418,9 @@
   int C = 0, T = 0, Hi = 0, Wi = 0, Ho = 0, Wo = 0, ld_out = 0, c_off = 0;
   PoolW pw{};
 };
+struct Step {
+  int op[2];
+};
 
 int sf_fail(int code, const char* fmt, ...) {
   char buf[768];
@@ -336,6 +439,7 @@
   bool finalized = false;
   std::map<std::string, HostTensor> host;
   std::vector<Op> ops;
+  std::vector<Step> steps;
   std::vector<size_t> buf_elems;
   std::vector<bf16_t*> bufs;
   bf16_t* d_w = nullptr;
@@ -367,7 +471,7 @@
   void need(int buf, size_t elems) {
     if (sf->buf_elems[buf] < elems) sf->buf_elems[buf] = elems;
   }
-  bool conv(const std::string& conv_name, const std::string& norm_name, int in_buf, int ld_in, int cin_eff, int Ti, int Hi, int Wi, int kt, int kh,
+  int conv(const std::string& conv_name, const std::string& norm_name, int in_buf, int ld_in, int cin_eff, int Ti, int Hi, int Wi, int kt, int kh,
             int kw, int st, int sh, int sw, int pt, int ph, int pw, int cout, int out_buf, int ld_out, int c_off, int res_buf, int ld_res, bool relu,
             int* To_, int* Ho_, int* Wo_, bool stem_pairs = false) {
     const HostTensor* W = get(conv_name + ".weight");
@@ -377,12 +481,12 @@
     const HostTensor* var = get(norm_name + ".running_var");
     const int To = (Ti + 2 * pt - kt) / st + 1, Ho = (Hi + 2 * ph - kh) / sh + 1, Wo = (Wi + 2 * pw - kw) / sw + 1;
     *To_ = To; *Ho_ = Ho; *Wo_ = Wo;
-    if (!W || !g || !be || !mu || !var) return false;
+    if (!W || !g || !be || !mu || !var) return -1;
     const int cin_real = W->shape.size() == 5 ? (int)W->shape[1] : -1;
     if (W->shape.size() != 5 || W->shape[0] != cout || (stem_pairs ? cin_real != 3 : cin_real != cin_eff) || W->shape[2] != kt || W->shape[3] != kh || W->shape[4] != kw ||
         (int)g->v.size() != cout || (int)be->v.size() != cout || (int)mu->v.size() != cout || (int)var->v.size() != cout) {
       if (missing.size() < 400) missing += (missing.empty() ? "" : ", ") + conv_name + " (bad shape)";
-      return false;
+      return -1;
     }
     const int taps = kt * kh * kw;
     const int kw_k = stem_pairs ? 4 : kw, taps_k = kt * kh * kw_k;
@@ -417,7 +521,7 @@
     need(out_buf, (size_t)op.rows_per_clip * ld_out);
     sf->flops_per_clip += 2.0 * op.rows_per_clip * cout * (double)taps * cin_real;
     sf->ops.push_back(op);
-    return true;
+    return (int)sf->ops.size() - 1;
   }
 };
 
@@ -426,6 +530,78 @@
     const int lo = i - k + 1 > 0 ? i - k + 1 : 0, hi = i < n - k ? i : n - k;
     w[i] = (float)(hi - lo + 1);
   }
+}
+
+ConvArgs bind_conv(const aigv_slowfast* sf, const Op& op, int clips) {
+  ConvArgs a = op.a;
+  a.in = sf->bufs[op.in_buf]; a.out = sf->bufs[op.out_buf]; a.res = op.res_buf >= 0 ? sf->bufs[op.res_buf] : nullptr;
+  a.w = sf->d_w + op.w_off; a.bias = sf->d_b + op.b_off;
+  a.rows = op.rows_per_clip * clips;
+  return a;
+}
+
+MaxPoolArgs bind_maxpool(const aigv_slowfast* sf, const Op& op, int clips) {
+  return MaxPoolArgs{sf->bufs[op.in_buf], sf->bufs[op.out_buf], op.C, op.Hi, op.Wi, op.Ho, op.Wo, op.ld_out, (long)clips * op.T * op.Ho * op.Wo * (op.C / 8)};
+}
+
+PoolArgs bind_pool(const aigv_slowfast* sf, const Op& op) {
+  return PoolArgs{sf->bufs[op.in_buf], op.T, op.Hi, op.Wi, op.C, op.ld_out, op.c_off, op.pw};
+}
+
+hipError_t run_step(const aigv_slowfast* sf, const Step& st, int clips, const void* frames, void* feature, hipStream_t s) {
+  const Op& op = sf->ops[st.op[0]];
+  const Op* op1 = st.op[1] >= 0 ? &sf->ops[st.op[1]] : nullptr;
+  switch (op.kind) {
+    case OP_REPACK: {
+      const long hw = (long)sf->H * sf->W, total = (long)clips * (sf->T + sf->Ts) * hw;
+      hipLaunchKernelGGL(sf_repack_kernel, dim3((unsigned)((total + 255) / 256)), dim3(256), 0, s, (const bf16_t*)frames, sf->T, sf->Ts, hw, sf->bufs[B_IN1],
+                         sf->bufs[B_IN0], sf->slow_idx, total);
+      return hipGetLastError();
+    }
+    case OP_CONV:
+      if (op1)
+        return launch_conv_pair(bind_conv(sf, op, clips), op.k_slices, bind_conv(sf, *op1, clips), op1->k_slices, s, sf->d_part, sf->part_floats);
+      return launch_conv(bind_conv(sf, op, clips), s, op.k_slices, sf->d_part, sf->part_floats);
+    case OP_MAXPOOL: {
+      MaxPoolPair q{};
+      q.m[0] = bind_maxpool(sf, op, clips);
+      q.nb0 = (unsigned)((q.m[0].total + 255) / 256);
+      unsigned nb = q.nb0;
+      if (op1) {
+        q.m[1] = bind_maxpool(sf, *op1, clips);
+        nb += (unsigned)((q.m[1].total + 255) / 256);
+      }
+      hipLaunchKernelGGL(sf_maxpool_kernel, dim3(nb), dim3(256), 0, s, q);
+      return hipGetLastError();
+    }
+    case OP_POOL: {
+      PoolPair q{};
+      q.p[0] = bind_pool(sf, op);
+      q.nb0 = (unsigned)((op.C + 31) / 32);
+      unsigned nb = q.nb0;
+      if (op1) {
+        q.p[1] = bind_pool(sf, *op1);
+        nb += (unsigned)((op1->C + 31) / 32);
+      }
+      hipLaunchKernelGGL(sf_pool_kernel, dim3(nb, clips), dim3(256), 0, s, q, (bf16_t*)feature);
+      return hipGetLastError();
+    }
+  }
+  return hipErrorInvalidValue;
+}
+
+int sf_forward(aigv_slowfast* sf, const void* frames, int clips, void* feature, void* stream, bool serial, const char* fn) {
+  if (!sf || !frames || !feature) return sf_fail(AIGV_ERR_ARG, "%s: null argument", fn);
+  if (!sf->finalized) return sf_fail(AIGV_ERR_STATE, "%s: call aigv_slowfast_finalize first", fn);
+  if (clips <= 0 || clips > sf->Bcap) return sf_fail(AIGV_ERR_ARG, "%s: %d clips, capacity %d", fn, clips, sf->Bcap);
+  if (hipSetDevice(sf->device) != hipSuccess) return sf_fail(AIGV_ERR_HIP, "%s: hipSetDevice(%d) failed", fn, sf->device);
+  const size_t n = serial ? sf->ops.size() : sf->steps.size();
+  for (size_t i = 0; i < n; ++i) {
+    const Step st = serial ? Step{{(int)i, -1}} : sf->steps[i];
+    const hipError_t e = run_step(sf, st, clips, frames, feature, (hipStream_t)stream);
+    if (e != hipSuccess) return sf_fail(e == hipErrorInvalidValue ? AIGV_ERR_ARG : AIGV_ERR_HIP, "%s: launch failed: %s", fn, hipGetErrorString(e));
+  }
+  return 0;
 }
 
 }
@@ -492,77 +668,95 @@
   if (sf->finalized) return 0;
   if (hipSetDevice(sf->device) != hipSuccess) return sf_fail(AIGV_ERR_HIP, "hipSetDevice failed");
   sf->ops.clear();
+  sf->steps.clear();
   sf->buf_elems.assign(B_COUNT, 0);
   sf->flops_per_clip = 0;
   Builder bd{sf, {}, {}, {}};
   const int T[2] = {sf->Ts, sf->T};
   const int IN[2] = {B_IN0, B_IN1}, STEM[2] = {B_STEM0, B_STEM1}, X[2][2] = {{B_X00, B_X01}, {B_X10, B_X11}}, A[2] = {B_A0, B_A1},
             Bq[2] = {B_B0, B_B1}, S[2] = {B_S0, B_S1};
+  bool ok = true;
+  auto pair = [&](int i0, int i1) {
+    ok &= i0 >= 0 && i1 >= 0;
+    sf->steps.push_back(Step{{i0, i1}});
+  };
+  auto single = [&](int i) {
+    ok &= i >= 0;
+    sf->steps.push_back(Step{{i, -1}});
+  };
   {
     Op op; op.kind = OP_REPACK;
     sf->ops.push_back(op);
+    single((int)sf->ops.size() - 1);
     bd.need(B_IN0, (size_t)sf->Ts * sf->H * sf->W * 4);
     bd.need(B_IN1, (size_t)sf->T * sf->H * sf->W * 4);
   }
-  bool ok = true;
   int h = 0, w = 0, to = 0;
   int ld[2] = {64 + 16, 8};
+  int stem_op[2], pool_op[2];
   for (int p = 0; p < 2; ++p) {
     const int kt = p ? 5 : 1, cout = p ? 8 : 64;
     const std::string pre = "0.multipathway_blocks." + std::to_string(p);
-    ok &= bd.conv(pre + ".conv", pre + ".norm", IN[p], 8, 8, T[p], sf->H, sf->W, kt, 7, 7, 1, 2, 2, kt / 2, 3, 3, cout, STEM[p], cout, 0, -1, 0, true, &to, &h, &w, true);
+    stem_op[p] = bd.conv(pre + ".conv", pre + ".norm", IN[p], 8, 8, T[p], sf->H, sf->W, kt, 7, 7, 1, 2, 2, kt / 2, 3, 3, cout, STEM[p], cout, 0, -1, 0, true, &to, &h,
+                         &w, true);
     Op mp; mp.kind = OP_MAXPOOL;
     mp.in_buf = STEM[p]; mp.out_buf = X[p][0]; mp.C = cout; mp.T = T[p]; mp.Hi = h; mp.Wi = w;
     mp.Ho = (h + 2 - 3) / 2 + 1; mp.Wo = (w + 2 - 3) / 2 + 1; mp.ld_out = ld[p];
     bd.need(X[p][0], (size_t)T[p] * mp.Ho * mp.Wo * ld[p]);
     sf->ops.push_back(mp);
+    pool_op[p] = (int)sf->ops.size() - 1;
     if (p == 1) { h = mp.Ho; w = mp.Wo; }
   }
+  pair(stem_op[0], stem_op[1]);
+  pair(pool_op[0], pool_op[1]);
   int sp_h = h, sp_w = w;
-  ok &= bd.conv("0.multipathway_fusion.conv_fast_to_slow", "0.multipathway_fusion.norm", X[1][0], 8, 8, T[1], sp_h, sp_w, 7, 1, 1, 4, 1, 1, 3, 0, 0, 16,
-                X[0][0], ld[0], 64, -1, 0, true, &to, &h, &w);
+  single(bd.conv("0.multipathway_fusion.conv_fast_to_slow", "0.multipathway_fusion.norm", X[1][0], 8, 8, T[1], sp_h, sp_w, 7, 1, 1, 4, 1, 1, 3, 0, 0, 16,
+                 X[0][0], ld[0], 64, -1, 0, true, &to, &h, &w));
   if (to != T[0]) return sf_fail(AIGV_ERR_ARG, "fast->slow fusion yields %d frames, slow pathway has %d", to, T[0]);
   int cur[2] = {0, 0};
   int cin[2] = {80, 8};
   static const int depths[4] = {3, 4, 6, 3};
   for (int s = 0; s < 4; ++s) {
-    int out_h = sp_h, out_w = sp_w;
+    int inner[2], cout[2], ld_out[2], kt_a[2];
     for (int p = 0; p < 2; ++p) {
-      const int inner = (p ? 8 : 64) << s, cout = inner * 4;
-      const int fuse_ch = (s < 3 && p == 0) ? 2 * (32 << s) : 0;
-      const int ld_out = cout + fuse_ch;
-      const int kt_a = (p == 1 || s >= 2) ? 3 : 1;
-      int bh = sp_h, bw = sp_w;
-      for (int blk = 0; blk < depths[s]; ++blk) {
-        const int stv = (blk == 0 && s > 0) ? 2 : 1;
+      inner[p] = (p ? 8 : 64) << s; cout[p] = inner[p] * 4;
+      ld_out[p] = cout[p] + ((s < 3 && p == 0) ? 2 * (32 << s) : 0);
+      kt_a[p] = (p == 1 || s >= 2) ? 3 : 1;
+    }
+    int bh = sp_h, bw = sp_w;
+    for (int blk = 0; blk < depths[s]; ++blk) {
+      const int stv = (blk == 0 && s > 0) ? 2 : 1;
+      int role[2][4] = {{-1, -1, -1, -1}, {-1, -1, -1, -1}};
+      int h2 = 0, w2 = 0;
+      for (int p = 0; p < 2; ++p) {
         const std::string pre = std::to_string(s + 1) + ".multipathway_blocks." + std::to_string(p) + ".res_blocks." + std::to_string(blk) + ".";
         const int xin = X[p][cur[p]], xout = X[p][cur[p] ^ 1];
-        const int c_in = blk == 0 ? cin[p] : cout, ld_in = blk == 0 ? ld[p] : ld_out;
-        int t1, h1, w1, h2, w2;
+        const int c_in = blk == 0 ? cin[p] : cout[p], ld_in = blk == 0 ? ld[p] : ld_out[p];
+        int t1, h1, w1;
         int res_buf = xin, res_ld = ld_in;
         if (blk == 0) {
-          ok &= bd.conv(pre + "branch1_conv", pre + "branch1_norm", xin, ld_in, c_in, T[p], bh, bw, 1, 1, 1, 1, stv, stv, 0, 0, 0, cout, S[p], cout, 0, -1, 0,
-                        false, &t1, &h1, &w1);
-          res_buf = S[p]; res_ld = cout;
+          role[p][0] = bd.conv(pre + "branch1_conv", pre + "branch1_norm", xin, ld_in, c_in, T[p], bh, bw, 1, 1, 1, 1, stv, stv, 0, 0, 0, cout[p], S[p], cout[p],
+                               0, -1, 0, false, &t1, &h1, &w1);
+          res_buf = S[p]; res_ld = cout[p];
         }
-        ok &= bd.conv(pre + "branch2.conv_a", pre + "branch2.norm_a", xin, ld_in, c_in, T[p], bh, bw, kt_a, 1, 1, 1, 1, 1, kt_a / 2, 0, 0, inner, A[p], inner, 0,
-                      -1, 0, true, &t1, &h1, &w1);
-        ok &= bd.conv(pre + "branch2.conv_b", pre + "branch2.norm_b", A[p], inner, inner, T[p], bh, bw, 1, 3, 3, 1, stv, stv, 0, 1, 1, inner, Bq[p], inner, 0, -1,
-                      0, true, &t1, &h2, &w2);
-        ok &= bd.conv(pre + "branch2.conv_c", pre + "branch2.norm_c", Bq[p], inner, inner, T[p], h2, w2, 1, 1, 1, 1, 1, 1, 0, 0, 0, cout, xout, ld_out, 0, res_buf,
-                      res_ld, true, &t1, &h1, &w1);
-        bh = h2; bw = w2;
+        role[p][1] = bd.conv(pre + "branch2.conv_a", pre + "branch2.norm_a", xin, ld_in, c_in, T[p], bh, bw, kt_a[p], 1, 1, 1, 1, 1, kt_a[p] / 2, 0, 0,
+                             inner[p], A[p], inner[p], 0, -1, 0, true, &t1, &h1, &w1);
+        role[p][2] = bd.conv(pre + "branch2.conv_b", pre + "branch2.norm_b", A[p], inner[p], inner[p], T[p], bh, bw, 1, 3, 3, 1, stv, stv, 0, 1, 1, inner[p],
+                             Bq[p], inner[p], 0, -1, 0, true, &t1, &h2, &w2);
+        role[p][3] = bd.conv(pre + "branch2.conv_c", pre + "branch2.norm_c", Bq[p], inner[p], inner[p], T[p], h2, w2, 1, 1, 1, 1, 1, 1, 0, 0, 0, cout[p],
+                             xout, ld_out[p], 0, res_buf, res_ld, true, &t1, &h1, &w1);
         cur[p] ^= 1;
       }
-      cin[p] = ld_out; ld[p] = ld_out;
-      out_h = bh; out_w = bw;
-    }
-    sp_h = out_h; sp_w = out_w;
+      for (int r = blk == 0 ? 0 : 1; r < 4; ++r) pair(role[0][r], role[1][r]);
+      bh = h2; bw = w2;
+    }
+    for (int p = 0; p < 2; ++p) { cin[p] = ld_out[p]; ld[p] = ld_out[p]; }
+    sp_h = bh; sp_w = bw;
     if (s < 3) {
       const int cf = 32 << s, cs = 256 << s;
       const std::string pre = std::to_string(s + 1) + ".multipathway_fusion";
-      ok &= bd.conv(pre + ".conv_fast_to_slow", pre + ".norm", X[1][cur[1]], cf, cf, T[1], sp_h, sp_w, 7, 1, 1, 4, 1, 1, 3, 0, 0, 2 * cf, X[0][cur[0]], ld[0], cs,
-                    -1, 0, true, &to, &h, &w);
+      single(bd.conv(pre + ".conv_fast_to_slow", pre + ".norm", X[1][cur[1]], cf, cf, T[1], sp_h, sp_w, 7, 1, 1, 4, 1, 1, 3, 0, 0, 2 * cf, X[0][cur[0]], ld[0],
+                     cs, -1, 0, true, &to, &h, &w));
     }
   }
   if (!ok) return sf_fail(AIGV_ERR_STATE, "aigv_slowfast_finalize: missing or mis-shaped tensors: %s%s", bd.missing.c_str(), bd.missing.size() >= 400 ? " ..." : "");
@@ -583,6 +777,7 @@
     for (int x = 0; x < sp_w; ++x) op.pw.x[x] = tx[x] / nx;
     sf->ops.push_back(op);
   }
+  pair((int)sf->ops.size() - 2, (int)sf->ops.size() - 1);
   auto dmalloc = [&](void** p, size_t bytes) { return hipMalloc(p, bytes ? bytes : 16); };
   if (dmalloc((void**)&sf->d_w, bd.w.size() * 2) != hipSuccess || dmalloc((void**)&sf->d_b, bd.b.size() * 4) != hipSuccess)
     return sf_fail(AIGV_ERR_ALLOC, "aigv_slowfast_finalize: hipMalloc of %zu weight bytes failed", bd.w.size() * 2);
@@ -595,11 +790,16 @@
     if (hipMalloc((void**)&sf->bufs[i], bytes) != hipSuccess) return sf_fail(AIGV_ERR_ALLOC, "aigv_slowfast_finalize: hipMalloc(%zu) failed", bytes);
     if (hipMemset(sf->bufs[i], 0, bytes) != hipSuccess) return sf_fail(AIGV_ERR_HIP, "hipMemset failed");
   }
+  for (Op& op : sf->ops)
+    if (op.kind == OP_CONV) op.k_slices = conv_k_slices(op.rows_per_clip, op.a.CoutPad, op.a.Kp);
   size_t need = 0;
-  for (Op& op : sf->ops) {
-    if (op.kind != OP_CONV) continue;
-    op.k_slices = conv_k_slices(op.rows_per_clip, op.a.CoutPad, op.a.Kp);
-    if (op.k_slices > 1) need = std::max(need, (size_t)op.k_slices * op.rows_per_clip * sf->Bcap * op.a.Cout);
+  for (const Step& st : sf->steps) {
+    size_t n = 0;
+    for (int i : st.op) {
+      const Op* op = i >= 0 ? &sf->ops[i] : nullptr;
+      if (op && op->kind == OP_CONV && op->k_slices > 1) n += (size_t)op->k_slices * op->rows_per_clip * sf->Bcap * op->a.Cout;
+    }
+    need = std::max(need, n);
   }
   sf->part_floats = need;
   if (sf->part_floats && hipMalloc((void**)&sf->d_part, sf->part_floats * sizeof(float)) != hipSuccess)
@@ -612,46 +812,11 @@
 double aigv_slowfast_flops_per_clip(const aigv_slowfast* sf) { return sf ? sf->flops_per_clip : 0.0; }
 
 int aigv_slowfast_forward(aigv_slowfast* sf, const void* frames_nchw_bf16, int clips, void* feature_bf16, void* stream) {
-  if (!sf || !frames_nchw_bf16 || !feature_bf16) return sf_fail(AIGV_ERR_ARG, "aigv_slowfast_forward: null argument");
-  if (!sf->finalized) return sf_fail(AIGV_ERR_STATE, "aigv_slowfast_forward: call aigv_slowfast_finalize first");
-  if (clips <= 0 || clips > sf->Bcap) return sf_fail(AIGV_ERR_ARG, "aigv_slowfast_forward: %d clips, capacity %d", clips, sf->Bcap);
-  if (hipSetDevice(sf->device) != hipSuccess) return sf_fail(AIGV_ERR_HIP, "aigv_slowfast_forward: hipSetDevice(%d) failed", sf->device);
-  hipStream_t s = (hipStream_t)stream;
-  for (const Op& op : sf->ops) {
-    hipError_t e = hipSuccess;
-    switch (op.kind) {
-      case OP_REPACK: {
-        const long hw = (long)sf->H * sf->W, total = (long)clips * (sf->T + sf->Ts) * hw;
-        hipLaunchKernelGGL(sf_repack_kernel, dim3((unsigned)((total + 255) / 256)), dim3(256), 0, s, (const bf16_t*)frames_nchw_bf16, sf->T, sf->Ts, hw,
-                           sf->bufs[B_IN1], sf->bufs[B_IN0], sf->slow_idx, total);
-        e = hipGetLastError();
-        break;
-      }
-      case OP_CONV: {
-        ConvArgs a = op.a;
-        a.in = sf->bufs[op.in_buf]; a.out = sf->bufs[op.out_buf]; a.res = op.res_buf >= 0 ? sf->bufs[op.res_buf] : nullptr;
-        a.w = sf->d_w + op.w_off; a.bias = sf->d_b + op.b_off;
-        a.rows = op.rows_per_clip * clips;
-        e = launch_conv(a, s, op.k_slices, sf->d_part, sf->part_floats);
-        break;
-      }
-      case OP_MAXPOOL: {
-        const long total = (long)clips * op.T * op.Ho * op.Wo * (op.C / 8);
-        hipLaunchKernelGGL(sf_maxpool_kernel, dim3((unsigned)((total + 255) / 256)), dim3(256), 0, s, sf->bufs[op.in_buf], op.C, op.Hi, op.Wi, op.Ho, op.Wo,
-                           sf->bufs[op.out_buf], op.ld_out, total);
-        e = hipGetLastError();
-        break;
-      }
-      case OP_POOL: {
-        hipLaunchKernelGGL(sf_pool_kernel, dim3((op.C + 31) / 32, clips), dim3(256), 0, s, sf->bufs[op.in_buf], op.T, op.Hi, op.Wi, op.C, op.pw,
-                           (bf16_t*)feature_bf16, op.ld_out, op.c_off);
-        e = hipGetLastError();
-        break;
-      }
-    }
-    if (e != hipSuccess) return sf_fail(e == hipErrorInvalidValue ? AIGV_ERR_ARG : AIGV_ERR_HIP, "aigv_slowfast_forward: launch failed: %s", hipGetErrorString(e));
-  }
-  return 0;
+  return sf_forward(sf, frames_nchw_bf16, clips, feature_bf16, stream, false, "aigv_slowfast_forward");
+}
+
+int aigv_slowfast_forward_serial(aigv_slowfast* sf, const void* frames_nchw_bf16, int clips, void* feature_bf16, void* stream) {
+  return sf_forward(sf, frames_nchw_bf16, clips, feature_bf16, stream, true, "aigv_slowfast_forward_serial");
 }
 
 int aigv_op_conv3d(const void* x, int ld_in, int Cin, int B, const int* dims, const void* w_packed, int Kp, const float* bias, int Cout, const void* res,
diff --git a/aigv-assessor_amd/native.py b/aigv-assessor_amd/native.py
--- a/aigv-assessor_amd/native.py
+++ b/aigv-assessor_amd/native.py
@@ -70,6 +70,7 @@
     "aigv_slowfast_load_weight": (_I, [_P, C.c_char_p, _P, C.POINTER(C.c_int64), _I, _I]),
     "aigv_slowfast_finalize": (_I, [_P]),
     "aigv_slowfast_forward": (_I, [_P, _P, _I, _P, _P]),
+    "aigv_slowfast_forward_serial": (_I, [_P, _P, _I, _P, _P]),
     "aigv_slowfast_flops_per_clip": (C.c_double, [_P]),
     "aigv_op_conv3d": (_I, [_P, _I, _I, _I, C.POINTER(_I), _P, _I, _P, _I, _P, _I, _P, _I, _I, _I, _P]),
     "aigv_set_precision": (_I, [_P, _I]),
diff --git a/aigv-assessor_amd/slowfast.py b/aigv-assessor_amd/slowfast.py
--- a/aigv-assessor_amd/slowfast.py
+++ b/aigv-assessor_amd/slowfast.py
@@ -108,7 +108,7 @@
     def _native(self, device: torch.device, clips: int, T: int, H: int, W: int):
         return self.prepare(device, clips, T, H, W)
 
-    def features(self, pixel_values: torch.Tensor, clips: int) -> torch.Tensor:
+    def features(self, pixel_values: torch.Tensor, clips: int, serial: bool = False) -> torch.Tensor:
         if not pixel_values.is_cuda:
             raise RuntimeError("SlowFastR50 runs on the GPU only (no CPU fallback)")
         if pixel_values.dim() != 4 or pixel_values.shape[1] != 3 or clips <= 0 or pixel_values.shape[0] % clips:
@@ -117,7 +117,8 @@
         x = pixel_values.to(torch.bfloat16).contiguous()
         lib, h = self._native(x.device, clips, T, H, W)
         out = torch.empty((clips, FEATURE_DIM), dtype=torch.bfloat16, device=x.device)
-        native.check(lib.aigv_slowfast_forward(h, x.data_ptr(), clips, out.data_ptr(), native.stream_ptr()))
+        fwd = lib.aigv_slowfast_forward_serial if serial else lib.aigv_slowfast_forward
+        native.check(fwd(h, x.data_ptr(), clips, out.data_ptr(), native.stream_ptr()))
         return out
 
     def flops_per_clip(self) -> float:
diff --git a/include/aigv_amd.h b/include/aigv_amd.h
--- a/include/aigv_amd.h
+++ b/include/aigv_amd.h
@@ -180,6 +180,7 @@
 int aigv_slowfast_load_weight(aigv_slowfast* sf, const char* name, const void* host_data, const int64_t* shape, int ndim, int dtype);
 int aigv_slowfast_finalize(aigv_slowfast* sf);
 int aigv_slowfast_forward(aigv_slowfast* sf, const void* frames_nchw_bf16, int clips, void* feature_bf16, void* stream);
+int aigv_slowfast_forward_serial(aigv_slowfast* sf, const void* frames_nchw_bf16, int clips, void* feature_bf16, void* stream);
 double aigv_slowfast_flops_per_clip(const aigv_slowfast* sf);
 int aigv_op_conv3d(const void* x, int ld_in, int Cin, int B, const int* dims, const void* w_packed, int Kp, const float* bias, int Cout,
                    const void* res, int ld_res, void* out, int ld_out, int c_off, int relu, void* stream);
```

Result: no change. 33.50 (-0.2%).
